# fedemagnani/optimization-solvers

Measured on AMD Instinct MI355X. Metric: BFGS iterations/sec on n-dim convex quadratic (f64) at 1/2/4/8 MI355X, higher is better.
Workload: dtype f64

## Files before the change

include/qn_hip.h:

```cpp
#ifndef QN_HIP_H
#define QN_HIP_H

#include <stddef.h>
#include <stdint.h>

#ifdef __cplusplus
extern "C" {
#endif

#define QN_ABI_VERSION 5

typedef enum {
    QN_OK = 0,
    QN_MAX_ITER_REACHED = 1,
    QN_OUT_OF_DOMAIN = 2,
    QN_ERROR_INPUT_PARAMS = 3,
    QN_ABNORMAL_TERMINATION = 4
} qn_status;

const char* qn_status_string(int status);
const char* qn_last_error_message(void);
int qn_abi_version(void);

typedef struct qn_context qn_context;
// ... 84 lines not shown
enum { QN_BFGS = 0, QN_DFP = 1, QN_GRADIENT_DESCENT = 2, QN_NEWTON = 3 ,
       QN_SR1 = 4 ,
       QN_SPG = 5 ,
       QN_PROJECTED_GRADIENT = 6 ,
       QN_PROJECTED_NEWTON = 7 ,
       QN_SPECTRAL_PROJECTED_NEWTON = 8 ,
       QN_BROYDEN = 9 ,
       QN_COORDINATE_DESCENT = 10 ,
       QN_PNORM_DESCENT = 11 ,
       QN_LBFGS = 12  };
#define QN_LBFGS_MAX_M 32
typedef struct qn_solver qn_solver;

int qn_solver_create(qn_context* ctx, int method, double tol, const double* x0_host, size_t n, qn_solver** out);
void qn_solver_destroy(qn_solver* s);
int qn_solver_set_bounds(qn_solver* s, const double* lower_bound_host, const double* upper_bound_host);
int qn_solver_set_spg_lambdas(qn_solver* s, double lambda_min, double lambda_max);
int qn_solver_spg_lambda(qn_solver* s, double* out, int* is_some);
int qn_solver_newton_factorisations(qn_solver* s, size_t* out);
int qn_solver_set_lbfgs_memory(qn_solver* s, size_t m);
int qn_solver_lbfgs_state(qn_solver* s, size_t* m, size_t* stored, double* gamma, size_t* resets);
int qn_solver_set_inverse_p(qn_solver* s, const double* p_colmajor_host);
int qn_solver_get_inverse_p(qn_solver* s, double* out_colmajor_host);
int qn_solver_reset(qn_solver* s, const double* x0_host);

typedef void (*qn_callback_fn)(void* user, qn_solver* solver);

int qn_minimize(qn_solver* s, qn_linesearch* ls, const qn_oracle* oracle, size_t max_iter_solver,
                size_t max_iter_line_search, qn_callback_fn callback, void* callback_user);

int qn_compute_step_len(qn_context* ctx, qn_linesearch* ls, const double* x_k_host, double f_k, const double* g_k_host,
                        const double* direction_host, size_t n, const qn_oracle* oracle, size_t max_iter, double* step_out);

size_t qn_solver_n(const qn_solver* s);
size_t qn_solver_k(const qn_solver* s);
int qn_solver_set_k(qn_solver* s, size_t k);
double qn_solver_tol(const qn_solver* s);
int qn_solver_get_x(qn_solver* s, double* out_host);
int qn_solver_set_x(qn_solver* s, const double* x_host);
int qn_solver_s_norm(qn_solver* s, double* out, int* is_some);
int qn_solver_y_norm(qn_solver* s, double* out, int* is_some);
int qn_solver_next_iterate_too_close(qn_solver* s, int* out);
int qn_solver_gradient_next_iterate_too_close(qn_solver* s, int* out);
int qn_solver_decrement_squared(qn_solver* s, double* out, int* is_some);
int qn_solver_get_inv_hessian(qn_solver* s, double* out_colmajor_host, int all_ranks);
int qn_solver_set_inv_hessian(qn_solver* s, const double* h_colmajor_host);
int qn_solver_compute_direction(qn_solver* s, const double* g_host, double* d_host);
int qn_solver_secant_update(qn_solver* s, const double* s_host, const double* y_host);

#define QN_TRACE_LS_MODIFIED (1 << 30)
typedef struct {
    double f, gnorm, t, s_norm, y_norm;
    int32_t n_evals;
    int32_t ls_iters;
    int32_t ls_cases;
    int32_t updated;
} qn_trace_rec;
int qn_solver_set_trace(qn_solver* s, size_t cap, int with_x);
int qn_solver_get_trace(qn_solver* s, qn_trace_rec* out_host, size_t cap, size_t* len, double* x_trace_host);

typedef struct {
    uint64_t iterations;
    uint64_t oracle_calls;
    uint64_t oracle_evals;
    uint64_t h_passes;
    uint64_t h_bytes;
    uint64_t obj_bytes;
    uint64_t launches;
    uint64_t host_syncs;
    double   t_hpass_ms, t_eval_ms, t_ctl_ms, t_comm_ms;
    uint64_t n_hpass_timed, n_eval_timed, n_ctl_timed, n_comm_timed;
    uint64_t matrix_bytes_per_pass;
    uint64_t total_minimize_calls, total_iterations, total_oracle_calls, total_oracle_evals, total_h_passes, total_h_bytes,
        total_obj_bytes;
    uint32_t path;
    uint32_t _pad;
    double   t_hreduce_ms, t_ereduce_ms;
    uint64_t n_hreduce_timed, n_ereduce_timed;
    uint64_t total_xchg_vector, total_xchg_scalar;
    double   t_newton_ms;
    uint64_t n_newton_timed;
    uint64_t newton_lu_sync_timeouts;
    uint64_t fast_machine_steps;
} qn_stats;
#define QN_PATH_FUSED 1u
#define QN_PATH_SYM 2u
#define QN_PATH_SYM_GENERIC 4u
#define QN_PATH_PIPELINED 8u
#define QN_PATH_SYM2 16u
#define QN_PATH_TILES1 32u
#define QN_PATH_VECTOR 64u
#define QN_PATH_PNEWTON 128u
#define QN_PATH_RANK1 256u
#define QN_PATH_PNORM 512u
#define QN_PATH_LBFGS 1024u
int qn_solver_get_stats(qn_solver* s, qn_stats* out);
int qn_solver_set_profiling(qn_solver* s, int on);
int qn_solver_set_sync_mode(qn_solver* s, int sync);
int qn_solver_set_tiling(qn_solver* s, int rows_per_block, int col_splits);
typedef enum {
    QN_OPT_GENERIC_KERNELS = 1,
    QN_OPT_DEFERRED_UPDATE_STEP = 2,
    QN_OPT_SYMMETRIC_STORAGE = 3,
    QN_OPT_SECOND_GENERATION = 4,
    QN_OPT_FOLDED_ACCEPT_REDUCE = 5,
    QN_OPT_ROW_SLIVERS = 6,
    QN_OPT_EVAL_PAIR_INSTANCE = 7,
    QN_OPT_EVAL_MOVER_MULTIPLIER = 8,
    QN_OPT_TAIL_REDUCE = 9,
    QN_OPT_BOUNDED_SECOND_GENERATION = 10,
    QN_OPT_NEWTON_PIVOTED_LU = 11,
    QN_OPT_LU_PER_COLUMN_PANEL = 12,
    QN_OPT_LU_LOOKAHEAD = 13,
    QN_OPT_LU_ONE_LAUNCH_PANEL = 14,
    QN_OPT_LU_FORCE_WAIT_EXPIRY = 15,
    QN_OPT_CHUNKS_PER_TRIP = 16,
    QN_OPT_LU_SPLIT_ROLE_A = 17,
    QN_OPT_LU_SPLIT_MIN_ROWS = 18,
    QN_OPT_BTB_PROJECT_IN_EVAL = 19,
    QN_OPT_EVAL_ZIGZAG = 20,
    QN_OPT_TOUCH_H_ROWS = 21,
    QN_OPT_TOUCH_Q_ROWS = 22,
    QN_OPT_PNEWTON_REUSE_FACTOR = 23,
    QN_OPT_PNORM_NONTEMPORAL = 24,
    QN_OPT_PNORM_ROWS_PER_WAVE = 25,
    QN_OPT_LBFGS_UNIT_SCALING = 26,
    QN_OPT_MACHINE_FAST_STEPS = 27
} qn_option;
int qn_solver_set_option(qn_solver* s, int option, int value);

int qn_dev_alloc(qn_context* ctx, size_t bytes, void** out_dev);
int qn_dev_free(qn_context* ctx, void* dev);
int qn_h2d(qn_context* ctx, void* dst_dev, const void* src_host, size_t bytes);
int qn_d2h(qn_context* ctx, void* dst_host, const void* src_dev, size_t bytes);
int qn_gemv(qn_context* ctx, const double* a_dev, size_t ld, size_t nrows, size_t ncols, const double* x_dev, double* y_dev);
int qn_rank2_update(qn_context* ctx, double* h_dev, size_t ld, size_t row0, size_t nrows, size_t n, const double* s_dev,
                    const double* u_dev, double c_ss, double c_su, double c_uu);
int qn_axpy(qn_context* ctx, size_t n, const double* x_dev, double t, const double* d_dev, double* out_dev);
int qn_dot(qn_context* ctx, size_t n, const double* a_dev, const double* b_dev, double* out_host);
int qn_nrm2(qn_context* ctx, size_t n, const double* a_dev, double* out_host);

#ifdef __cplusplus
}
#endif
#endif
```

optimization-solvers_amd/_abi.py:

```python
import ctypes as C
import os

_HERE = os.path.dirname(os.path.abspath(__file__))
LIB_PATH = os.environ.get("QN_HIP_LIB") or os.path.join(_HERE, "lib", "libqn_hip.so")

OK, MAX_ITER_REACHED, OUT_OF_DOMAIN, ERROR_INPUT_PARAMS, ABNORMAL_TERMINATION = range(5)
LS_MORETHUENTE, LS_BACKTRACKING, LS_MORETHUENTE_B, LS_BACKTRACKING_B, LS_GLL_QUADRATIC = 0, 1, 2, 3, 4
LS_NO_SEARCH = 5
LS_STRONG_WOLFE = 6
ORACLE_HOST, ORACLE_DEVICE_FN, ORACLE_OBJECTIVE = 0, 1, 2
BFGS, DFP, GRADIENT_DESCENT, NEWTON, SR1, SPG, PROJECTED_GRADIENT, PROJECTED_NEWTON, SPECTRAL_PROJECTED_NEWTON = 0, 1, 2, 3, 4, 5, 6, 7, 8
BROYDEN = 9
COORDINATE_DESCENT, PNORM_DESCENT = 10, 11
LBFGS = 12
LBFGS_MAX_M = 32
UNIQUE_ID_BYTES = 128

dp = C.POINTER(C.c_double)


class LineSearchStruct(C.Structure):
    _fields_ = [("kind", C.c_int32), ("_pad", C.c_int32),
                ("c1", C.c_double), ("c2", C.c_double), ("t_min", C.c_double), ("t_max", C.c_double),
                ("delta_min", C.c_double), ("delta", C.c_double), ("delta_max", C.c_double),
                ("bt_c1", C.c_double), ("bt_beta", C.c_double),
                ("lower_bound_host", C.c_void_p), ("upper_bound_host", C.c_void_p)]


HOST_ORACLE_FN = C.CFUNCTYPE(C.c_int, C.c_void_p, dp, C.c_size_t, dp, dp)
DEVICE_ORACLE_FN = C.CFUNCTYPE(C.c_int, C.c_void_p, C.c_void_p, C.c_void_p, C.c_size_t, C.c_void_p, C.c_void_p)
CALLBACK_FN = C.CFUNCTYPE(None, C.c_void_p, C.c_void_p)
HOST_HESSIAN_FN = C.CFUNCTYPE(C.c_int, C.c_void_p, dp, C.c_size_t, dp)
HOST_ALLGATHER_FN = C.CFUNCTYPE(C.c_int, C.c_void_p, dp, dp, C.c_size_t)


class OracleStruct(C.Structure):
    _fields_ = [("kind", C.c_int32), ("memoize", C.c_int32),
                ("host_fn", C.c_void_p), ("host_user", C.c_void_p),
                ("device_fn", C.c_void_p), ("device_user", C.c_void_p),
                ("objective", C.c_void_p), ("host_hessian_fn", C.c_void_p)]


class TraceRec(C.Structure):
    _fields_ = [("f", C.c_double), ("gnorm", C.c_double), ("t", C.c_double), ("s_norm", C.c_double), ("y_norm", C.c_double),
                ("n_evals", C.c_int32), ("ls_iters", C.c_int32), ("ls_cases", C.c_int32), ("updated", C.c_int32)]


class Stats(C.Structure):
    _fields_ = [("iterations", C.c_uint64), ("oracle_calls", C.c_uint64), ("oracle_evals", C.c_uint64),
                ("h_passes", C.c_uint64), ("h_bytes", C.c_uint64), ("obj_bytes", C.c_uint64),
                ("launches", C.c_uint64), ("host_syncs", C.c_uint64),
                ("t_hpass_ms", C.c_double), ("t_eval_ms", C.c_double), ("t_ctl_ms", C.c_double), ("t_comm_ms", C.c_double),
                ("n_hpass_timed", C.c_uint64), ("n_eval_timed", C.c_uint64), ("n_ctl_timed", C.c_uint64), ("n_comm_timed", C.c_uint64),
                ("matrix_bytes_per_pass", C.c_uint64),
                ("total_minimize_calls", C.c_uint64), ("total_iterations", C.c_uint64), ("total_oracle_calls", C.c_uint64),
                ("total_oracle_evals", C.c_uint64), ("total_h_passes", C.c_uint64), ("total_h_bytes", C.c_uint64),
                ("total_obj_bytes", C.c_uint64), ("path", C.c_uint32), ("_pad", C.c_uint32),
                ("t_hreduce_ms", C.c_double), ("t_ereduce_ms", C.c_double), ("n_hreduce_timed", C.c_uint64), ("n_ereduce_timed", C.c_uint64),
                ("total_xchg_vector", C.c_uint64), ("total_xchg_scalar", C.c_uint64),
                ("t_newton_ms", C.c_double), ("n_newton_timed", C.c_uint64), ("newton_lu_sync_timeouts", C.c_uint64),
                ("fast_machine_steps", C.c_uint64)]


PATH_FUSED, PATH_SYM, PATH_SYM_GENERIC, PATH_PIPELINED, PATH_SYM2, PATH_TILES1, PATH_VECTOR, PATH_PNEWTON = 1, 2, 4, 8, 16, 32, 64, 128
PATH_RANK1 = 256
PATH_PNORM = 512
PATH_LBFGS = 1024


SYMBOLS = [
    ("qn_status_string", C.c_char_p, [C.c_int]),
    ("qn_last_error_message", C.c_char_p, []),
    ("qn_abi_version", C.c_int, []),
    ("qn_device_count", C.c_int, [C.POINTER(C.c_int)]),
    ("qn_context_create", C.c_int, [C.c_int, C.POINTER(C.c_void_p)]),
    ("qn_comm_unique_id", C.c_int, [C.c_void_p]),
    ("qn_context_create_sharded", C.c_int, [C.c_int, C.c_int, C.c_int, C.c_void_p, C.POINTER(C.c_void_p)]),
    ("qn_context_create_sharded_host_exchange", C.c_int, [C.c_int, C.c_int, C.c_int, C.c_void_p, C.c_void_p, C.POINTER(C.c_void_p)]),
    ("qn_context_destroy", None, [C.c_void_p]),
    ("qn_partition", C.c_int, [C.c_size_t, C.c_int, C.POINTER(C.c_size_t), C.POINTER(C.c_size_t)]),
    ("qn_comm_selftest", C.c_int, [C.c_void_p]),
    ("qn_context_comm_check", C.c_int, [C.c_void_p]),
    ("qn_context_exchange_probe", C.c_int, [C.c_void_p, C.c_size_t, C.c_int, C.POINTER(C.c_double)]),
    ("qn_context_event_bracket_overhead", C.c_int, [C.c_void_p, C.c_int, C.POINTER(C.c_double)]),
    ("qn_context_synchronize", C.c_int, [C.c_void_p]),
    ("qn_context_rank", C.c_int, [C.c_void_p]),
    ("qn_context_world", C.c_int, [C.c_void_p]),
    ("qn_context_stream", C.c_void_p, [C.c_void_p]),
    ("qn_context_set_host_exchange_async", C.c_int, [C.c_void_p, C.c_int]),
    ("qn_context_set_trial_vector_exchange", C.c_int, [C.c_void_p, C.c_int]),
    ("qn_context_set_allreduce", C.c_int, [C.c_void_p, C.c_int]),
    ("qn_morethuente_default", None, [C.POINTER(LineSearchStruct)]),
    ("qn_morethuente_with_deltas", C.c_int, [C.POINTER(LineSearchStruct), C.c_double, C.c_double, C.c_double]),
    ("qn_morethuente_with_t_min", C.c_int, [C.POINTER(LineSearchStruct), C.c_double]),
    ("qn_morethuente_with_t_max", C.c_int, [C.POINTER(LineSearchStruct), C.c_double]),
    ("qn_morethuente_with_c1", C.c_int, [C.POINTER(LineSearchStruct), C.c_double]),
    ("qn_morethuente_with_c2", C.c_int, [C.POINTER(LineSearchStruct), C.c_double]),
    ("qn_backtracking_new", None, [C.POINTER(LineSearchStruct), C.c_double, C.c_double]),
    ("qn_morethuente_b_new", None, [C.POINTER(LineSearchStruct)]),
    ("qn_backtracking_b_new", None, [C.POINTER(LineSearchStruct), C.c_double, C.c_double, C.c_void_p, C.c_void_p]),
    ("qn_linesearch_with_lower_bound", None, [C.POINTER(LineSearchStruct), C.c_void_p]),
    ("qn_linesearch_with_upper_bound", None, [C.POINTER(LineSearchStruct), C.c_void_p]),
    ("qn_nosearch_new", None, [C.POINTER(LineSearchStruct)]),
    ("qn_gll_quadratic_new", None, [C.POINTER(LineSearchStruct), C.c_double, C.c_size_t]),
    ("qn_gll_quadratic_with_sigmas", None, [C.POINTER(LineSearchStruct), C.c_double, C.c_double]),
    ("qn_strong_wolfe_new", None, [C.POINTER(LineSearchStruct), C.c_double, C.c_double]),
    ("qn_strong_wolfe_with_xtol", C.c_int, [C.POINTER(LineSearchStruct), C.c_double]),
    ("qn_quadratic_create", C.c_int, [C.c_void_p, C.c_size_t, dp, dp, C.POINTER(C.c_void_p)]),
    ("qn_quadratic_create_synthetic", C.c_int, [C.c_void_p, C.c_size_t, C.c_uint64, dp, dp, C.POINTER(C.c_void_p)]),
    ("qn_logsumexp_create", C.c_int, [C.c_void_p, C.c_size_t, C.c_size_t, dp, dp, C.c_double, C.POINTER(C.c_void_p)]),
    ("qn_objective_destroy", None, [C.c_void_p]),
    ("qn_objective_eval", C.c_int, [C.c_void_p, dp, dp, dp]),
    ("qn_objective_get_rows", C.c_int, [C.c_void_p, C.c_size_t, C.c_size_t, dp]),
    ("qn_objective_hessian", C.c_int, [C.c_void_p, dp, dp]),
    ("qn_solver_create", C.c_int, [C.c_void_p, C.c_int, C.c_double, dp, C.c_size_t, C.POINTER(C.c_void_p)]),
    ("qn_solver_destroy", None, [C.c_void_p]),
    ("qn_solver_reset", C.c_int, [C.c_void_p, dp]),
    ("qn_solver_set_bounds", C.c_int, [C.c_void_p, dp, dp]),
    ("qn_solver_set_inverse_p", C.c_int, [C.c_void_p, dp]),
    ("qn_solver_get_inverse_p", C.c_int, [C.c_void_p, dp]),
    ("qn_solver_set_spg_lambdas", C.c_int, [C.c_void_p, C.c_double, C.c_double]),
    ("qn_solver_spg_lambda", C.c_int, [C.c_void_p, dp, C.POINTER(C.c_int)]),
    ("qn_solver_newton_factorisations", C.c_int, [C.c_void_p, C.POINTER(C.c_size_t)]),
    ("qn_solver_set_lbfgs_memory", C.c_int, [C.c_void_p, C.c_size_t]),
    ("qn_solver_lbfgs_state", C.c_int, [C.c_void_p, C.POINTER(C.c_size_t), C.POINTER(C.c_size_t), dp, C.POINTER(C.c_size_t)]),
    ("qn_minimize", C.c_int, [C.c_void_p, C.POINTER(LineSearchStruct), C.POINTER(OracleStruct), C.c_size_t, C.c_size_t, C.c_void_p, C.c_void_p]),
    ("qn_compute_step_len", C.c_int, [C.c_void_p, C.POINTER(LineSearchStruct), dp, C.c_double, dp, dp, C.c_size_t, C.POINTER(OracleStruct), C.c_size_t,
                             C.POINTER(C.c_double)]),
    ("qn_solver_n", C.c_size_t, [C.c_void_p]),
    ("qn_solver_k", C.c_size_t, [C.c_void_p]),
    ("qn_solver_set_k", C.c_int, [C.c_void_p, C.c_size_t]),
    ("qn_solver_tol", C.c_double, [C.c_void_p]),
    ("qn_solver_get_x", C.c_int, [C.c_void_p, dp]),
    ("qn_solver_set_x", C.c_int, [C.c_void_p, dp]),
    ("qn_solver_s_norm", C.c_int, [C.c_void_p, dp, C.POINTER(C.c_int)]),
    ("qn_solver_y_norm", C.c_int, [C.c_void_p, dp, C.POINTER(C.c_int)]),
    ("qn_solver_next_iterate_too_close", C.c_int, [C.c_void_p, C.POINTER(C.c_int)]),
    ("qn_solver_gradient_next_iterate_too_close", C.c_int, [C.c_void_p, C.POINTER(C.c_int)]),
    ("qn_solver_decrement_squared", C.c_int, [C.c_void_p, dp, C.POINTER(C.c_int)]),
    ("qn_solver_get_inv_hessian", C.c_int, [C.c_void_p, dp, C.c_int]),
    ("qn_solver_set_inv_hessian", C.c_int, [C.c_void_p, dp]),
    ("qn_solver_compute_direction", C.c_int, [C.c_void_p, dp, dp]),
    ("qn_solver_secant_update", C.c_int, [C.c_void_p, dp, dp]),
    ("qn_solver_set_trace", C.c_int, [C.c_void_p, C.c_size_t, C.c_int]),
# ... 37 lines not shown
```

optimization-solvers_amd/csrc/qn_ctl.h:

```cpp
#pragma once
#include <stdint.h>

enum QnPhase : int32_t {
    QN_PH_IDLE = 0,
    QN_PH_REQ_EVAL = 1,
    QN_PH_REQ_HPASS = 2,
    QN_PH_ITER_DONE = 3,
    QN_PH_DONE = 4,
    QN_PH_REQ_HPASS_EVAL = 7,
    QN_PH_REQ_VEC = 8,
    QN_PH_REQ_NEWTON = 6,
    QN_PH_REQ_DIR = 9,
    QN_PH_REQ_STEEP = 10
};

enum QnReqKind : int32_t { QN_REQ_X = 0 , QN_REQ_T = 1  };

enum QnState : int32_t {
    QN_ST_BEGIN = 0,
    QN_ST_LOOP_TOP,
    QN_ST_AFTER_EVALX,
    QN_ST_CHECK,
    QN_ST_AFTER_DIR,
    QN_ST_LS_BEGIN,
    QN_ST_MT_LOOP,
    QN_ST_MT_AFTER_T,
    QN_ST_MT_AFTER_TL,
    QN_ST_MT_AFTER_TU,
    QN_ST_MT_FINISH,
    QN_ST_BT_LOOP,
    QN_ST_BT_AFTER,
    QN_ST_AFTER_LS,
    QN_ST_AFTER_NEXT,
    QN_ST_AFTER_U,
    QN_ST_ITER_END,
    QN_ST_AFTER_NEWTON,
    QN_ST_LS_ONLY,
    QN_ST_AFTER_STEEP
};

#define QN_METHOD_BROYDEN 9
#define QN_METHOD_CD 10
#define QN_METHOD_PNORM 11
#define QN_LS_KIND_NOSEARCH 5
#define QN_LS_MODIFIED_BIT (1 << 30)

struct QnTraceRec {
    double f, gnorm, t, s_norm, y_norm;
    int32_t n_evals, ls_iters, ls_cases, updated;
};

struct QnCtl {
    double tol;
    int64_t max_iter, max_iter_ls;
    int32_t method, ls_kind, memoize, callback_mode;
    double mt_c1, mt_c2, mt_tmin, mt_tmax, mt_delta;
    double bt_c1, bt_beta;
    int64_t trace_cap;
    int32_t trace_x;
    int32_t small_n;

    int32_t phase, state, status, after_state;
    int64_t k;
    int32_t has_s_norm, has_y_norm;
    double s_norm, y_norm;
    double f_k;
    double gd0;
    double gnorm;
    double gg;
    int32_t gg_valid, xtrace_done;
    int32_t have_cur_eval;
    int32_t have_dir;

    int32_t fused, xc, sc, dir_mode, gd0_valid;
    int32_t no_defer;
    int32_t warm;
    int32_t defer_u;
    int32_t sym2;
    int32_t serviced;
    int32_t ev_par;
    int32_t ev_kind;
    double ev_t;
    double dir_ug, dir_sg;
    double st_gd0, st_yy, st_ys, st_gg, st_ss, st_dnf;
    double hp_yu, hp_ug, hp_sg;
    double hp_den;

    int32_t bounded, req_project, last_projected;
    int32_t ls_only;
    double mtb_cand;
    double bt_diff2;

    int32_t has_dec;
    int32_t s2_dir;
    double dec;

    int32_t req_kind, req_need_vectors;
    double req_t;
    int32_t hp_nrhs, hp_lazy;

    int32_t pending;
    int32_t spec_tiles;
    double c_ss, c_su, c_uu;

    double f_e, gd_e;
    int32_t last_valid, d_finite;
    double last_t, f_last, gd_last;

    int64_t ls_i;
    double t, tl, tu, ls_result;
    int32_t use_mod, conv;
    double phi_t_f, phi_t_g, psi_t_f, psi_t_g;
    double sel_f_tl, sel_g_tl, sel_f_t, sel_g_t;
    double ys;

    double tr_f, tr_gnorm;
    int32_t tr_n_evals, tr_ls_iters, tr_ls_cases, tr_ndigits, tr_updated;
    int32_t dir_ready;

    uint64_t n_oracle_calls, n_oracle_evals, n_hpasses, n_hpass_rw, n_iterations;
    uint64_t n_fast_steps;
};
```

optimization-solvers_amd/csrc/qn_ctl_step.hip.h:

```cpp
#pragma once

#ifdef QN_CTL_STAMPS
#define QN_STAMP(id) do { if (tid == 0 && V.dbg) V.dbg[stamp_base + (id)] = wall_clock64(); } while (0)
#else
#define QN_STAMP(id) do { } while (0)
#endif

#define QN_TILE_IDX(base)                                        \
    int idx[4];                                                  \
    bool ok[4];                                                  \
    _Pragma("unroll") for (int u_ = 0; u_ < 4; ++u_) {           \
        const int i_ = (base) + u_ * tpb + tid;                  \
        ok[u_] = i_ < n_pad;                                     \
        idx[u_] = ok[u_] ? i_ : 0;                               \
    }

template <int NP>
__device__ __forceinline__ void ctl_sum_partials(const double* __restrict__ part, int world, int nblk, double* lds, int wave0 = 0) {
    const int lane = threadIdx.x & 63, wave = (int)(threadIdx.x >> 6) - wave0, nw = (int)(blockDim.x >> 6) - wave0;
    if (wave < 0) return;
    for (int k = wave; k < NP; k += nw) {
        const double acc = qn_partial_col_sum(part, world, nblk, NP, k, lane);
        if (lane == 0) lds[k] = acc;
    }
}

__device__ __forceinline__ void qn_keepalive(double v) { asm volatile("" ::"v"(v)); }

__device__ __forceinline__ bool qn_check_is_scalar(const QnCtl& c) {
    return c.method != 2 && c.method != QN_METHOD_CD && c.method != QN_METHOD_PNORM && (c.small_n || c.gg_valid || c.method == 3);
}


template <int LEAN>
__device__ __forceinline__ void qn_st_begin(QnCtl& c) {
    c.k = 0;
    if (!c.warm) { c.have_cur_eval = 0; c.have_dir = 0; c.last_valid = 0; c.gg_valid = 0; }
    else c.last_valid = 0;
    c.n_oracle_calls = 0; c.n_oracle_evals = 0; c.n_hpasses = 0; c.n_hpass_rw = 0; c.n_iterations = 0;
    c.status = -1;
    c.state = QN_ST_LOOP_TOP;
}

template <int LEAN>
__device__ __forceinline__ void qn_st_loop_top(QnCtl& c) {
    if (!(c.max_iter > c.k)) {
        c.status = 1;
        c.phase = QN_PH_DONE;
    } else {
        c.tr_n_evals = 0; c.tr_ls_iters = 0; c.tr_ls_cases = 0; c.tr_ndigits = 0; c.tr_updated = 0;
        c.ls_result = NAN;
        c.n_oracle_calls++;
        c.tr_n_evals++;
        if (c.memoize && c.have_cur_eval) {
            c.state = QN_ST_CHECK;
        } else {
            c.req_kind = QN_REQ_X; c.req_t = 0.0; c.req_need_vectors = 1;
            c.after_state = QN_ST_AFTER_EVALX;
            c.phase = QN_PH_REQ_EVAL;
        }
    }
}

template <int LEAN>
__device__ __forceinline__ bool qn_st_after_evalx(QnCtl& c) {
    if (!LEAN && !c.fused) return false;
    c.f_k = c.f_e;
    c.gg = c.st_gg; c.gg_valid = 1;
    c.have_cur_eval = c.memoize;
    c.have_dir = 0;
    c.state = QN_ST_CHECK;
    return true;
}

template <int LEAN>
__device__ __forceinline__ bool qn_st_after_dir(QnCtl& c) {
    if (!LEAN && !c.fused) return false;
    c.n_hpasses++;
    if (c.pending) c.n_hpass_rw++;
    c.pending = 0;
    c.dir_mode = 0;
    c.gd0_valid = 0; c.d_finite = 0; c.last_valid = 0;
    c.state = QN_ST_LS_BEGIN;
    if (LEAN == 2 && c.s2_dir) { c.dir_ready = 0; c.after_state = QN_ST_LS_BEGIN; c.phase = QN_PH_REQ_DIR; }
    return true;
}

template <int LEAN>
__device__ __forceinline__ bool qn_st_after_next(QnCtl& c) {
    if (!LEAN && !c.fused) return false;
    c.s_norm = sqrt(c.st_ss); c.has_s_norm = 1;
    c.y_norm = sqrt(c.st_yy); c.has_y_norm = 1;
    c.ys = c.st_ys;
    c.gg = c.st_gg; c.gg_valid = 1;
    c.f_k = c.f_e;
    c.xc ^= 1;
    c.have_cur_eval = c.memoize;
    c.have_dir = 0;
    c.last_valid = 0;
    if (c.s_norm < c.tol || c.y_norm < c.tol) {
        c.state = QN_ST_ITER_END;
    } else {
        c.hp_lazy = 1; c.hp_nrhs = 2;
        const double fk = c.f_k;
        const bool will_continue = (c.k + 1 < c.max_iter) && !(isnan(fk) || isinf(fk)) && !(sqrt(c.gg) < c.tol);
        if (!LEAN && will_continue && !c.callback_mode && !c.no_defer && !c.sym2) {
            c.defer_u = 1;
            c.tr_updated = 1;
            c.have_dir = 1; c.gd0_valid = 0; c.d_finite = 0;
            c.state = QN_ST_ITER_END;
        } else {
            c.after_state = QN_ST_AFTER_U;
            c.phase = QN_PH_REQ_HPASS;
        }
    }
    return true;
}

template <int LEAN>
__device__ __forceinline__ bool qn_st_after_u(QnCtl& c) {
    if (!LEAN && !c.fused) return false;
    const double yu = c.hp_yu;
    double c_ss, c_su, c_uu;
    qn_update_coeffs(c.method, c.ys, yu, c_ss, c_su, c_uu, c.hp_den);
    c.c_ss = c_ss; c.c_su = c_su; c.c_uu = c_uu;
    c.n_hpasses++;
    if (c.pending) c.n_hpass_rw++;
    c.pending = 1;
    c.sc ^= 1;
    c.dir_mode = 1; c.dir_ug = c.hp_ug; c.dir_sg = c.hp_sg;
    c.gd0_valid = 0; c.d_finite = 0;
    c.have_dir = 1;
    if (LEAN == 2) c.dir_ready = 0;
    c.tr_updated = 1;
    c.state = QN_ST_ITER_END;
    return true;
}

template <int LEAN>
__device__ __forceinline__ bool qn_st_check(QnCtl& c, const QnVecs& V, double* small_scratch) {
    const int n = V.n, n_pad = V.n_pad;
    if (!LEAN && !qn_check_is_scalar(c)) return false;
    if (!LEAN && c.method == 3) {
        c.gnorm = c.gg_valid ? sqrt(c.gg) : NAN; c.tr_f = c.f_k; c.tr_gnorm = c.gnorm;
        const double f = c.f_k;
        if (isnan(f) || isinf(f)) { c.status = 2; c.phase = QN_PH_DONE; }
        else if (c.has_dec && c.dec * 0.5 < c.tol) { c.status = 0; c.phase = QN_PH_DONE; }
        else { c.after_state = QN_ST_AFTER_NEWTON; c.phase = QN_PH_REQ_NEWTON; }
        return true;
    }
    double gnorm, gd0 = c.gd0;
    int d_finite = c.d_finite;
    if (!LEAN && c.small_n) {
        gnorm = sqrt(ref_dot(V.g, V.g, n));
        small_direction(V.H, n_pad, n, V.g, V.d, small_scratch, V.x, c.bounded ? V.lb : nullptr, c.bounded ? V.ub : nullptr);
        if (c.ls_kind == 2) {
            double cand = INFINITY;
            for (int i = 0; i < n; ++i) {
                const double di = V.d[i];
                double v = INFINITY;
                if (di > 0.0) v = (V.lub[i] - V.x[i]) / di; else if (di < 0.0) v = (V.llb[i] - V.x[i]) / di;
                cand = fmin(v, cand);
            }
            c.mtb_cand = cand;
        }
        gd0 = ref_dot(V.g, V.d, n);
        d_finite = 1;
        for (int i = 0; i < n; ++i) d_finite &= isfinite(V.d[i]) ? 1 : 0;
    } else {
        gnorm = sqrt(c.gg);
    }
    c.gnorm = gnorm; c.tr_f = c.f_k; c.tr_gnorm = gnorm;
    const double f = c.f_k;
    if (isnan(f) || isinf(f)) {
        c.status = 2; c.phase = QN_PH_DONE;
    } else if ((c.has_s_norm && c.s_norm < c.tol) || (c.has_y_norm && c.y_norm < c.tol) || (gnorm < c.tol)) {
        c.status = 0; c.phase = QN_PH_DONE;
    } else if (!LEAN && c.small_n) {
        c.gd0 = gd0; c.d_finite = d_finite; c.last_valid = 0;
        c.state = QN_ST_LS_BEGIN;
    } else if (c.have_dir) {
        c.state = QN_ST_LS_BEGIN;
        if (LEAN == 2 && c.s2_dir) {
            if (!c.dir_ready) { c.after_state = QN_ST_LS_BEGIN; c.phase = QN_PH_REQ_DIR; }
            else if (c.s2_dir & 2) c.mt_tmax = fmin(c.mt_tmax, c.mtb_cand);
        }
    } else {
        c.hp_nrhs = 1; c.hp_lazy = 0;
        c.after_state = QN_ST_AFTER_DIR;
        c.phase = QN_PH_REQ_HPASS;
    }
    return true;
}

template <int LEAN>
__device__ __forceinline__ void qn_st_ls_begin(QnCtl& c) {
    c.ls_i = 0;
    if (!LEAN && c.ls_kind == QN_LS_KIND_NOSEARCH) { c.ls_result = 1.0; c.state = QN_ST_AFTER_LS; return; }
    if (!LEAN && c.ls_kind == 2) c.mt_tmax = fmin(c.mt_tmax, c.mtb_cand);
    if (c.ls_kind == 0 || (!LEAN && c.ls_kind == 2)) {
        c.use_mod = 0; c.conv = 0;
        c.t = fmin(fmax(1.0, c.mt_tmin), c.mt_tmax);
        c.tl = c.mt_tmin; c.tu = c.mt_tmax;
        c.state = QN_ST_MT_LOOP;
    } else {
        c.t = 1.0;
        c.state = QN_ST_BT_LOOP;
    }
}

template <int LEAN>
// ... 757 lines not shown
```

optimization-solvers_amd/csrc/qn_host_launch.hip.h:

```cpp
#pragma once
struct Run;
static int r1_enqueue_req(qn_solver* s);
static int steep_enqueue_req(qn_solver* s);
static int enqueue_newton(qn_solver* s, const qn_oracle* o, qn_objective* obj);

static int check_oracle(qn_context* c, size_t n, const qn_oracle* o, qn_objective** obj) {
    *obj = nullptr;
    if (o->kind == QN_ORACLE_HOST) return o->host_fn ? QN_OK : fail(QN_ERROR_INPUT_PARAMS, "host oracle is null");
    if (o->kind == QN_ORACLE_DEVICE_FN) return o->device_fn ? QN_OK : fail(QN_ERROR_INPUT_PARAMS, "device oracle is null");
    if (o->kind != QN_ORACLE_OBJECTIVE) return fail(QN_ERROR_INPUT_PARAMS, "unknown oracle kind");
    if (!o->objective) return fail(QN_ERROR_INPUT_PARAMS, "objective is null");
    if (o->objective->ctx != c || o->objective->n != n) return fail(QN_ERROR_INPUT_PARAMS, "objective does not match the solver");
    *obj = o->objective;
    return QN_OK;
}
static void stats_add_totals(qn_solver* s) {
    s->stats.total_minimize_calls++;
    s->stats.total_iterations += s->stats.iterations; s->stats.total_oracle_calls += s->stats.oracle_calls; s->stats.total_oracle_evals += s->stats.oracle_evals;
    s->stats.total_h_passes += s->stats.h_passes; s->stats.total_h_bytes += s->stats.h_bytes; s->stats.total_obj_bytes += s->stats.obj_bytes;
}
static int xchg_sum_or_gather(qn_context* c, double* buf, size_t cnt) { return c->use_allreduce ? exchange_sum(c, buf, cnt) : exchange(c, buf, cnt); }

struct Run {
    qn_solver* s;
// ... 256 lines not shown
                a.parity = (int)(r.s2_launches & 1);
                hipLaunchKernelGGL(s2sh_vsumt_kernel, dim3(a.nb), dim3(QN_S2_TPB), 0, c->stream, a);
                HIPCHK(hipGetLastError());
                s->stats.launches++;
            }
            ProfScope ps(s, KC_COMM);
            const XchgItem items[2] = {{half, cnt}, {s->symsh_xg, (size_t)s->T.n_pad}};
            c->n_xchg_scalar++;
            QNCHK(exchange_group(c, items, 2));
            return QN_OK;
        }
        ProfScope ps(s, KC_COMM);
        c->n_xchg_scalar++;
        QNCHK(xchg_sum_or_gather(c, half, cnt));
    }
    return QN_OK;
}
static int s2_do_vec(Run& r) {
    qn_solver* s = r.s;
    qn_context* c = s->ctx;
    if (r.s2.sh_world > 1 && c->trial_vector && !r.gobj) return s2_launch(r, QN_S2_VECD);
    if (r.s2.sh_world > 1) {
        QNCHK(s2_launch(r, QN_S2_VSUM));
        {
            ProfScope ps(s, KC_COMM);
            c->n_xchg_vector++;
            if (r.gobj) QNCHK(exchange(c, r.obj->lgall, (size_t)s->T.n_pad));
            else QNCHK(xchg_sum_or_gather(c, s->symsh_xg, (size_t)s->T.n_pad));
        }
        return s2_launch(r, QN_S2_VEC);
    }
    return s2_launch(r, r.s2.fold ? QN_S2_HTILE : QN_S2_VEC);
}
static int s2_do_hpass(Run& r, bool tiles) {
    qn_solver* s = r.s;
    qn_context* c = s->ctx;
    if (r.gobj && r.s2.sh_world == 1) {
        if (!tiles) return fail(QN_ABNORMAL_TERMINATION, "sym2 (generic objective): tiles marked done without their launch");
        QNCHK(s2_launch(r, QN_S2_GHT_A));
        QNCHK(s2g_enqueue_tiles(r));
        return s2_launch(r, QN_S2_HREDUCE);
    }
    if (tiles && r.tiles1) {
        QNCHK(s2_launch(r, QN_S2_GHT_A));
        QNCHK(s2g_enqueue_tiles(r));
    } else if (tiles) QNCHK(s2_launch(r, QN_S2_HTILE));
    if (r.s2.tred) return QN_OK;
    if (r.s2.sh_world > 1) {
        QNCHK(s2_launch(r, QN_S2_HSUM));
        ProfScope ps(s, KC_COMM);
        c->n_xchg_vector++;
        QNCHK(xchg_sum_or_gather(c, s->symsh_xg, 2 * (size_t)s->T.n_pad));
    }
    return s2_launch(r, QN_S2_HREDUCE);
}

static int s2_wait_report(Run& r, unsigned long long seq) {
    qn_solver* s = r.s;
    volatile unsigned long long* flag = s->hrep_flag;
    for (uint64_t spins = 0;; ++spins) {
        if (__atomic_load_n(flag, __ATOMIC_ACQUIRE) == seq) break;
        if ((spins & 0xfff) == 0xfff) {
            hipError_t e = hipStreamQuery(s->ctx->stream);
            if (e == hipSuccess) { if (__atomic_load_n(flag, __ATOMIC_ACQUIRE) == seq) break; return fail(QN_ABNORMAL_TERMINATION, "sym2: the batch ended without a report"); }
            if (e != hipErrorNotReady) return fail(QN_ABNORMAL_TERMINATION, std::string("sym2 batch: ") + hipGetErrorString(e));
        }
    }
    memcpy(s->hctl, s->hrep, sizeof(QnCtl));
    s->stats.host_syncs++;
    return QN_OK;
}

static int place_h(Run& r) {
    qn_solver* s = r.s;
    if (s->h_placed) return QN_OK;
    s->h_placed = true;
    const size_t np = s->T.n_pad, bytes = (size_t)s->T.rpr * np * sizeof(double);
    const char* sw = getenv("QN_H_PLACEMENT");
    if ((sw && atoi(sw) == 0) || s->ctx->world != 1 || bytes > ((size_t)330 << 20) || r.s2.fold) return QN_OK;
    hipStream_t st = s->ctx->stream;
    QnCtl* pc = s->hrep;
    memcpy(pc, s->hctl, sizeof(QnCtl));
    pc->phase = QN_PH_REQ_HPASS; pc->serviced = 0; pc->hp_nrhs = 1; pc->pending = 0; pc->after_state = QN_ST_AFTER_DIR; pc->sym2 = 1; pc->fused = 1;
    pc->spec_tiles = 0; pc->sc = 0; pc->xc = 0;
    PinnedBuf<QnCtl> pe;
    (void)pe.alloc(1, hipHostMallocMapped | hipHostMallocCoherent);
    if (pe) {
        memcpy(pe, s->hctl, sizeof(QnCtl));
        pe->phase = QN_PH_REQ_EVAL; pe->serviced = 0; pe->sym2 = 1; pe->fused = 1; pe->sc = 0; pe->xc = 0;
        pe->ev_kind = QN_REQ_T; pe->t = 1.0; pe->status = -1;
    }
    ScopedEvent e0, e1;
    if (hipEventCreate(&e0.e) != hipSuccess || hipEventCreate(&e1.e) != hipSuccess) { (void)hipGetLastError(); return QN_OK; }
    auto time_on = [&](double* H, float* out_us) -> int {
        QnS2Args a = r.s2;
        a.H = H; a.parity = 0; a.ctl_first = pc; a.rep_seq = 0;
        a.tred = 0;
        float t[6];
        for (int rep = 0; rep < 6; ++rep) {
            if (pe) {
                QnS2Args ae = a;
                ae.ctl_first = pe;
                for (int e = 0; e < 2; ++e) s2_launch_eval_plain(st, ae);
            }
            HIPCHK(hipEventRecord(e0.e, st));
            if (s->method == QN_BFGS) hipLaunchKernelGGL((s2_hpass_kernel<false, true, false>), dim3(a.G), dim3(QN_S2_TPB), 0, st, a);
            else hipLaunchKernelGGL((s2_hpass_kernel<false, false, false>), dim3(a.G), dim3(QN_S2_TPB), 0, st, a);
            HIPCHK(hipEventRecord(e1.e, st));
            HIPCHK(hipEventSynchronize(e1.e));
            float ms = 0.f;
            HIPCHK(hipEventElapsedTime(&ms, e0.e, e1.e));
            t[rep] = ms * 1e3f;
        }
        std::sort(t + 2, t + 6);
        *out_us = t[3];
        return QN_OK;
    };
    DevBuf<double> cand[2];
    struct Drain { hipStream_t st; ~Drain() { (void)hipStreamSynchronize(st); } } drained{st};
    float us[3] = {0.f, 0.f, 0.f};
    int ncand = 1, keep = 0;
    QNCHK(time_on(s->H, &us[0]));
    for (int k = 1; k < 3; ++k) {
        if (k == 2 && std::fabs(us[0] - us[1]) <= 0.06f * std::min(us[0], us[1])) break;
        if (cand[k - 1].alloc((size_t)s->T.rpr * np) != QN_OK) break;
        ++ncand;
        if (hipMemcpyAsync(cand[k - 1], s->H, bytes, hipMemcpyDeviceToDevice, st) != hipSuccess) return fail(QN_ABNORMAL_TERMINATION, "H placement: copy failed");
        QNCHK(time_on(cand[k - 1], &us[k]));
    }
    for (int k = 1; k < ncand; ++k)
        if (us[k] < 0.96f * us[keep]) keep = k;
    if (sw && atoi(sw) == 2) fprintf(stderr, "[qn] H placement: %d candidates, update kernel %.2f %.2f %.2f us, kept %d\n", ncand, us[0], us[1], us[2], keep);
    if (keep) {
        (void)hipStreamSynchronize(st);
        s->H = std::move(cand[keep - 1]);
        s->V.H = s->H;
        r.s2.H = s->H;
    }
    return QN_OK;
}

static int launch_ctl_mask(Run& r, int expect_mask) {
    qn_solver* s = r.s;
    ProfScope ps(s, KC_CTL);
    const bool hp = (expect_mask & ((1 << QN_PH_REQ_HPASS) | (1 << QN_PH_REQ_HPASS_EVAL))) != 0;
    const bool ev = (expect_mask & ((1 << QN_PH_REQ_EVAL) | (1 << QN_PH_REQ_HPASS_EVAL))) != 0;
    const dim3 blk(r.fused ? ((hp && ev) ? 768 : 576) : QN_CTL_TPB);
    QnVecs V = s->V;
    if (r.rank1) V.hcs = 1;
    if (r.oracle_tpl == QN_ORACLE_QUAD)
        hipLaunchKernelGGL(ctl_step_kernel<QN_ORACLE_QUAD>, dim3(1), blk, 0, s->ctx->stream, s->ctl, V, expect_mask);
    else
        hipLaunchKernelGGL(ctl_step_kernel<QN_ORACLE_GENERIC>, dim3(1), blk, 0, s->ctx->stream, s->ctl, V, expect_mask);
    s->stats.launches++;
    HIPCHK(hipGetLastError());
    return QN_OK;
}
static int launch_ctl(Run& r, int expect_phase) { return launch_ctl_mask(r, 1 << expect_phase); }

template <int R, int U>
static void launch_eval_fused(hipStream_t st, const QnEvalFusedArgs& a) {
    hipLaunchKernelGGL((quad_eval_fused_kernel<R, U>), dim3(a.T.rpr / R), dim3(QN_TPB), 0, st, a);
}
template <int R, int U>
static void launch_hpass_fused(hipStream_t st, const QnHPassFusedArgs& a) {
    hipLaunchKernelGGL((h_pass_fused_kernel<R, U>), dim3(a.T.rpr / R), dim3(QN_TPB), 0, st, a);
}
// ... 195 lines not shown
```

optimization-solvers_amd/csrc/qn_host_minimize.hip.h:

```cpp
#pragma once
static int vec_minimize(qn_solver* s, qn_linesearch* ls, const qn_oracle* o, size_t max_iter_solver, size_t max_iter_line_search,
                        qn_callback_fn callback, void* callback_user, int ls_only, double ls_f0);
static int vec_compute_step_len(qn_context* ctx, qn_linesearch* ls, const double* x_k_host, double f_k, const double* g_k_host,
                                const double* direction_host, size_t n, const qn_oracle* oracle, size_t max_iter, double* step_out);

static int plan_run(Run& r, qn_solver* s, qn_linesearch* ls, const qn_oracle* o, size_t max_iter_solver, size_t max_iter_line_search, double ls_f0) {
    qn_context* c = s->ctx;
    const qn_callback_fn callback = r.callback;
    const int ls_only = r.ls_only;
    if (ls->kind < QN_LS_MORETHUENTE || (ls->kind > QN_LS_BACKTRACKING_B && ls->kind != QN_LS_NO_SEARCH)) return fail(QN_ERROR_INPUT_PARAMS, "unknown line search");
    if (ls->kind == QN_LS_NO_SEARCH && s->method != QN_GRADIENT_DESCENT && s->method != QN_NEWTON && !steep_method(s->method))
        return fail(QN_ERROR_INPUT_PARAMS, "NoSearch pairs with GradientDescent, Newton, CoordinateDescent and PnormDescent only");
    if (s->method == QN_PNORM_DESCENT && !s->pnorm_set) return fail(QN_ERROR_INPUT_PARAMS, "PnormDescent: inverse_p has not been set (qn_solver_set_inverse_p)");
    if (steep_method(s->method)) QNCHK(steep_alloc(s));
    const bool ls_bounded = r.ls_bounded = ls->kind == QN_LS_MORETHUENTE_B || ls->kind == QN_LS_BACKTRACKING_B;
    if (ls_bounded || s->bounded) {
        QNCHK(bounds_alloc(s));
        if (ls_bounded) {
            QNCHK(bounds_upload(s, s->bounds_block + 2 * (size_t)s->T.n_pad, ls->lower_bound_host, -INFINITY));
            QNCHK(bounds_upload(s, s->bounds_block + 3 * (size_t)s->T.n_pad, ls->upper_bound_host, INFINITY));
        }
    }
    {
        std::vector<double> box;
        if (ls_bounded) {
            box.assign(2 * s->n, 0.0);
            for (size_t i = 0; i < s->n; ++i) { box[i] = ls->lower_bound_host ? ls->lower_bound_host[i] : -INFINITY; box[s->n + i] = ls->upper_bound_host ? ls->upper_bound_host[i] : INFINITY; }
        }
        s->ls_box_changed = ls->kind != s->last_ls_kind || box.size() != s->last_ls_box.size() ||
                            (!box.empty() && memcmp(box.data(), s->last_ls_box.data(), box.size() * sizeof(double)) != 0);
        s->last_ls_kind = ls->kind;
        s->last_ls_box.swap(box);
    }
    if (s->method == QN_NEWTON) {
        if (c->world > 1) return fail(QN_ERROR_INPUT_PARAMS, "Newton is single-GPU (SURVEY.md 8(f) row f2)");
        if (!(r.obj && (r.obj->kind == OBJ_QUADRATIC || r.obj->kind == OBJ_LOGSUMEXP)) && !(o->kind == QN_ORACLE_HOST && o->host_hessian_fn))
            return fail(QN_ERROR_INPUT_PARAMS, "Hessian not available in the oracle");
        QNCHK(newton_alloc(s));
    }

    QnCtl* h = s->hctl;
    h->tol = s->tol;
    h->max_iter = (int64_t)std::min<size_t>(max_iter_solver, (size_t)1 << 62);
    h->max_iter_ls = (int64_t)std::min<size_t>(max_iter_line_search, (size_t)1 << 62);
    h->method = s->method;
    h->ls_kind = ls->kind;
    h->memoize = o->memoize ? 1 : 0;
    h->callback_mode = callback ? 1 : 0;
    h->mt_c1 = ls->c1; h->mt_c2 = ls->c2; h->mt_tmin = ls->t_min; h->mt_tmax = ls->t_max; h->mt_delta = ls->delta;
    h->bt_c1 = ls->bt_c1; h->bt_beta = ls->bt_beta;
    h->trace_cap = (int64_t)s->trace_cap;
    h->trace_x = s->trace_x;
    h->bounded = s->bounded;
    h->req_project = 0; h->last_projected = 0; s->mtb_cand_keep = h->mtb_cand; h->mtb_cand = INFINITY;
    h->ls_only = ls_only;
    if (ls_only) { h->f_k = ls_f0; h->have_cur_eval = 0; h->have_dir = 0; h->last_valid = 0; }
    h->small_n = (s->n <= QN_SMALL_N && c->world == 1) ? 1 : 0;
    if (h->small_n && h->pending) QNCHK(flush_pending(s));
    const bool sym_base = s->T.n_pad >= 8 * QN_TB && !s->no_sym && !s->h_nonsym;
    const bool sym_ok = c->world == 1 && (s->T.n_pad % QN_TB) == 0 && sym_base;
    const bool symsh_ok = c->world > 1 && (s->T.rpr % QN_TB) == 0 && sym_base;
    const bool s2_shape = sym_ok && (size_t)s->T.n_pad == s->n && !s->no_sym2;
    const bool s2sh_shape = symsh_ok && (size_t)s->T.n_pad == s->n && !s->no_sym2 && c->world <= 64;
    const bool s2bnd_off = getenv("QN_S2_BND") && atoi(getenv("QN_S2_BND")) == 0;
    const bool s2_struct = !ls_only && s2_shape && r.obj && r.obj->q_symmetric && !s->no_s2bnd && !s2bnd_off;
    const bool s2b = (s->bounded || ls_bounded) && s2_struct;
    const bool sr1_s2 = s->method == QN_SR1 && s2_struct;
    r.fused = r.oracle_tpl == QN_ORACLE_QUAD && h->memoize && (s->method == QN_BFGS || s->method == QN_DFP || sr1_s2) && !callback && s->hcs == 1 &&
              s->qcs == 1 && !h->small_n && !s->no_fused && (!(s->bounded || ls_bounded) || s2b);
    r.gobj = r.obj && r.obj->kind == OBJ_LOGSUMEXP && r.obj->lse_kch && !r.obj->lse_two_pass && h->memoize && (s->method == QN_BFGS || s->method == QN_DFP) &&
             !callback && s->hcs == 1 && !h->small_n && !s->no_fused && !s->bounded && !ls_bounded && !ls_only &&
             (s2_shape || (s2sh_shape && (c->comm || c->host_xchg || c->host_async))) && !(getenv("QN_S2G") && atoi(getenv("QN_S2G")) == 0);
    if (r.gobj) r.fused = true;
    h->fused = r.fused ? 1 : 0;
    s->V.fused_hint = h->fused;
    r.sym = r.fused && (sym_ok || symsh_ok) && r.obj && (r.obj->q_symmetric || r.gobj);
    r.sym_generic = !r.fused && (sym_ok || symsh_ok) && s->H && s->hcs == 1 && (s->method == QN_BFGS || s->method == QN_DFP || s->method == QN_SR1);
    r.rank1 = s->method == QN_BROYDEN && !h->small_n;
    r.pnorm = s->method == QN_PNORM_DESCENT && !h->small_n;
    if (s->method == QN_BROYDEN && (r.fused || r.sym || r.sym_generic)) return fail(QN_ABNORMAL_TERMINATION, "Broyden on a symmetric-storage path");
    if ((r.sym || r.sym_generic) && c->world > 1) QNCHK(solver_alloc_symsh_lists(s));
    if (r.sym_generic) {
        if (c->world > 1) QNCHK(s->symsh_xg.ensure((size_t)c->world * 2 * s->T.n_pad, c->stream));
        const int nb = s->T.n_pad / QN_TB;
        QNCHK(s->sym_part.ensure((size_t)nb * nb * 2 * QN_TB, c->stream));
        s->sym_nb = nb;
    }
    r.sym2 = r.sym && (s2_shape || s2sh_shape);
    h->sym2 = r.sym2 ? 1 : 0;
    r.bnd = r.sym2 && (s->bounded || ls_bounded || s->method == QN_SR1);
    if ((s->bounded || ls_bounded) && r.fused && !r.bnd) return fail(QN_ABNORMAL_TERMINATION, "bounded run on a fused path that is not the second-generation one");
    if (s->method == QN_SR1 && r.fused && !r.sym2) return fail(QN_ABNORMAL_TERMINATION, "SR1 on a fused path that is not the second-generation one");
    h->s2_dir = r.bnd ? ((s->bounded ? 1 : 0) | (ls->kind == QN_LS_MORETHUENTE_B ? 2 : 0)) : 0;
    r.dirq = h->s2_dir != 0;
    r.btb = r.bnd && ls->kind == QN_LS_BACKTRACKING_B;
    r.proj = r.btb;
    if (r.bnd && ls->kind == QN_LS_MORETHUENTE_B) h->ls_kind = QN_LS_MORETHUENTE;
    {
        const size_t hhalf = c->world > 1 ? (size_t)s->T.rpr * s->T.n_pad * 8 / 2 : (size_t)s->T.n_pad * s->T.n_pad * 8 / 2;
        r.tiles1 = r.sym2 && !r.gobj && c->world > 1 && hhalf > ((size_t)320 << 20);
        if (r.sym2 && !r.gobj && getenv("QN_S2_GEN1_TILES")) r.tiles1 = atoi(getenv("QN_S2_GEN1_TILES")) != 0;
    }
    h->serviced = 0; h->ev_par = 0; h->ev_kind = QN_REQ_X; h->ev_t = 0.0; h->spec_tiles = 0;
    h->n_fast_steps = 0;
    h->defer_u = 0;
    h->no_defer = s->no_defer;
    if (!r.fused) QNCHK(fused_export(s));
    if (!(r.sym || r.sym_generic) || (s->h_diag_stale && (!r.sym2 || (r.gobj && c->world == 1) || r.tiles1))) QNCHK(ensure_full_h(s));
    if (r.fused) {
        QNCHK(solver_alloc_fused(s, r.sym));
        s->V.F.pworld = r.sym ? 1 : c->world;
        if (r.sym && c->world > 1) QNCHK(s->symsh_xg.ensure((size_t)c->world * 2 * s->T.n_pad, c->stream));
        s->V.F.b = r.gobj ? nullptr : r.obj->b;
        if (!s->fused_live) {
            const size_t vb = (size_t)s->T.n_pad * sizeof(double);
            HIPCHK(hipMemcpyAsync(s->V.F.X0, s->V.x, vb, hipMemcpyDeviceToDevice, c->stream));
            if (h->pending) {
                HIPCHK(hipMemcpyAsync(s->V.F.S0, s->V.sp, vb, hipMemcpyDeviceToDevice, c->stream));
                HIPCHK(hipMemcpyAsync(s->V.F.UN, s->V.up, vb, hipMemcpyDeviceToDevice, c->stream));
            }
            h->xc = 0; h->sc = 0;
        }
        h->warm = (s->fused_live && s->warm_obj != 0 && s->warm_obj == r.obj->serial && h->memoize && h->pending && !ls_only) ? 1 : 0;
        if (!h->warm) { h->dir_mode = 0; h->gd0_valid = 0; h->dir_ready = 0; }
        if (!r.bnd || s->ls_box_changed) h->dir_ready = 0;
        if (r.bnd && h->dir_ready) h->mtb_cand = s->mtb_cand_keep;
    } else {
        h->warm = 0;
    }
    h->phase = QN_PH_IDLE;
    h->status = -1;
    const bool can_pipeline = (r.oracle_tpl == QN_ORACLE_QUAD || r.gobj) && !callback && !(c->world > 1 && !c->comm && !c->host_async);
    r.sync = s->method == QN_NEWTON || s->method == QN_BROYDEN || steep_method(s->method) || s->sync_mode == 1 || (s->sync_mode == -1 && !(can_pipeline && o->memoize)) || !can_pipeline;
    return QN_OK;
}

static void s2_cache_policy(size_t half, int* nt, int* ntq) {
    if (2 * half <= ((size_t)230 << 20)) { *nt = 0; *ntq = 0; }
    else if (half <= ((size_t)320 << 20)) { *nt = 0; *ntq = 1; }
    else { *nt = 1; *ntq = 1; }
}

static int plan_s2_args(Run& r) {
    qn_solver* s = r.s;
    qn_context* c = s->ctx;
    QNCHK(solver_alloc_sym2(s));
    QnS2Args& a = r.s2;
    a.Q = r.obj->Q; a.H = s->H; a.n = (int)s->n; a.np = s->T.n_pad; a.nb = s->s2_nb; a.G = s->s2_G;
    a.item_ij = s->s2_items; a.maxk = s->s2_maxk; a.inorder = s->s2_inorder; a.F = s->V.F; a.part = s->sym_part;
    a.wgS = s->s2_wgS; a.trows = s->s2_trows; a.ctl2 = s->s2_ctl; a.partE = s->s2_partE;
    a.gw = r.gobj ? s->T.n_pad / 64 : 0;
    a.gmu = r.gobj ? r.obj->mu : 0.0;
    if (r.gobj && c->world > 1) QNCHK(s->s2_gws.ensure(80, c->stream));
    a.gws = s->s2_gws;
    if (r.gobj) QNCHK(s->s2_wgV.ensure((size_t)2 * s->s2_trows * QN_S2_ROW, c->stream));
    a.wgV = s->s2_wgV;
    if (r.gobj && a.gw > s->s2_trows) return fail(QN_ABNORMAL_TERMINATION, "sym2 (generic objective): more combine workgroups than table rows");
    a.fold = (s->s2_maxk <= 3 && s->s2_nb <= 32 && s->fold) ? 1 : 0;
    a.sl_first = s->s2_sl_first; a.sl_per = s->s2_sl_per;
    a.pair = (a.sl_per != 0 && s->s2_maxk == 2 && s->s2_inorder == 2 * s->s2_G && !s->no_pair) ? 1 : 0;
    if (a.sl_per && !s->h_sliver_whole) { QNCHK(ensure_full_h(s)); s->h_sliver_whole = true; }
    a.trace = s->V.trace; a.xtrace = s->V.xtrace;
    a.sh_world = c->world; a.sh_rank = c->rank; a.sh_ioff = c->rank * (s->T.rpr / QN_TB);
    a.sh_nsum = c->use_allreduce ? 1 : c->world;
    a.evS = s->s2_evS; a.xg = s->symsh_xg; a.sl_off = s->s2_sl_off; a.sl_idx = s->s2_sl_idx;
    if (c->world > 1 || r.gobj) { a.fold = 0; a.pair = 0; }
    {
        a.ring = (a.pair && s->ring && s->s2_nb * (s->s2_nb - 1) / 2 >= s->s2_G) ? 1 : 0;
        a.zig = (a.ring && s->zig) ? 1 : 0;
    }
    a.fast = (s->fast_steps && c->world == 1 && !r.gobj && !r.bnd) ? 1 : 0;
    a.projfold = (r.btb && a.pair && a.ring && !s->no_projfold) ? 1 : 0;
    if (a.projfold) r.proj = false;
    if (r.bnd) a.fold = 0;
    a.method = s->method;
    if (s->method == QN_SR1) a.fold = 0;
    a.lb = (r.bnd && s->bounded) ? s->V.lb : nullptr; a.ub = (r.bnd && s->bounded) ? s->V.ub : nullptr;
    a.llb = (r.bnd && r.ls_bounded) ? s->V.llb : nullptr; a.lub = (r.bnd && r.ls_bounded) ? s->V.lub : nullptr;
    if (r.tiles1) a.fold = 0;
    a.cnt = s->s2_cnt;
    a.cnt_stride = getenv("QN_S2_CNT_STRIDE") ? std::max(1, std::min(QN_S2_CNT_STRIDE, atoi(getenv("QN_S2_CNT_STRIDE")))) : QN_S2_CNT_STRIDE;
    const bool want_tred = getenv("QN_S2_TRED") ? atoi(getenv("QN_S2_TRED")) != 0 : s->tred;
    if (want_tred) QNCHK(s->s2_cnt.ensure((size_t)a.nb * QN_S2_CNT_STRIDE, c->stream));
    a.cnt = s->s2_cnt;
    a.tred = (c->world == 1 && !a.fold && !r.gobj && !r.tiles1 && s->s2_maxk <= QN_S2_TRED_MAXK && want_tred && s->method != QN_SR1) ? 1 : 0;
    {
        auto rows_ok = [](int v) { return v == 4 || v == 6 || v == 8 || v == 10 || v == 12 || v == 16; };
        const bool can = a.ring && !r.bnd && !a.fold && !a.tred && s->method != QN_SR1 && a.nb == 32 && a.G == 256;
        a.touch = (can && rows_ok(s->touch)) ? s->touch : 0;
        a.touchq = (can && rows_ok(s->touchq)) ? s->touchq : 0;
        a.touch_delay = std::max(0, std::min(512, s->touch_delay));
        a.touchq_delay = std::max(0, std::min(512, s->touchq_delay));
    }
    s2_cache_policy(c->world > 1 ? (size_t)s->T.rpr * s->T.n_pad * 8 / 2 : (size_t)s->T.n_pad * s->T.n_pad * 8 / 2, &a.nt, &a.ntq);
    if (getenv("QN_S2_NT")) a.nt = atoi(getenv("QN_S2_NT"));
    if (getenv("QN_S2_NTQ")) a.ntq = atoi(getenv("QN_S2_NTQ"));
    return QN_OK;
}

static int slots_needed(uint64_t evals, uint64_t iters, int cap) {
    return (int)std::min<uint64_t>((uint64_t)cap, std::max<uint64_t>(1, (evals + iters - 1) / iters));
}

static int pump_s2_sync(Run& r) {
    QnCtl* h = r.s->hctl;
    QNCHK(s2_launch(r, QN_S2_ADVANCE));
    for (;;) {
        QNCHK(s2_peek(r));
        const int ph = h->phase;
        if (ph == QN_PH_DONE) { r.status = h->status; return QN_OK; }
        const bool tiles_done = ph == QN_PH_REQ_HPASS && h->serviced == 1;
        if (h->serviced != 0 && !tiles_done) return fail(QN_ABNORMAL_TERMINATION, "sym2: request in an unexpected service state");
        if (ph == QN_PH_REQ_EVAL) QNCHK(s2_do_eval(r));
        else if (ph == QN_PH_REQ_VEC) QNCHK(s2_do_vec(r));
        else if (ph == QN_PH_REQ_DIR && r.bnd) QNCHK(s2_launch(r, QN_S2_DIR));
        else if (ph == QN_PH_REQ_HPASS) QNCHK(s2_do_hpass(r, !tiles_done));
        else return fail(QN_ABNORMAL_TERMINATION, "sym2: control block in an unexpected phase");
        QNCHK(s2_launch(r, QN_S2_ADVANCE));
    }
}

static int pump_s2_pipelined(Run& r) {
    qn_solver* s = r.s;
    qn_context* c = s->ctx;
    QnCtl* h = s->hctl;
    int slots = (r.ls->kind == QN_LS_MORETHUENTE) ? 2 : 4;
    const bool adaptive = r.s2.sh_world > 1 || r.gobj || r.bnd;
    if (adaptive) slots = s->s2_slots_hint ? s->s2_slots_hint : (r.gobj ? 1 : 2);
    bool first = true;
    uint64_t ev0 = 0, it0 = 0;
    unsigned long long seq = 0;
    for (;;) {
        if (!first) {
            QNCHK(s2_wait_report(r, seq));
            if (adaptive && h->n_iterations > it0) {
                uint64_t de = h->n_oracle_evals - ev0;
                if (it0 == 0 && !h->warm && de > 0) de -= 1;
                slots = slots_needed(de, h->n_iterations - it0, 4);
                s->s2_slots_hint = slots;
            }
            ev0 = h->n_oracle_evals; it0 = h->n_iterations;
            if (h->phase == QN_PH_DONE) { r.status = h->status; return QN_OK; }
        }
        int64_t remaining = h->max_iter - (first ? 0 : h->k);
        if (remaining < 1) remaining = 1;
        const int64_t periods = std::min<int64_t>(remaining + ((first && !h->warm) ? 1 : 0), 256);
        first = false;
        auto one_period = [&]() -> int {
            if (r.dirq) QNCHK(s2_launch(r, QN_S2_DIR));
            for (int e = 0; e < slots; ++e) QNCHK(s2_do_eval(r));
            if (r.btb) QNCHK(s2_launch(r, QN_S2_ADVANCE));
            if (!r.s2.fold && !(r.gobj && r.s2.sh_world == 1)) QNCHK(s2_do_vec(r));
            QNCHK(s2_do_hpass(r, true));
            return QN_OK;
        };
        int64_t p = 0;
        static const bool want_graph = getenv("QN_S2_GRAPH") && atoi(getenv("QN_S2_GRAPH")) != 0;
        if (want_graph && c->world == 1 && !r.gobj && !s->profiling && periods >= 3) {
            QNCHK(one_period()); ++p;
            const uint64_t l0 = r.s2_launches;
            if ((l0 & 1) != 0) { QNCHK(one_period()); ++p; }
            if (periods - p >= 2) {
                const uint64_t lbase = r.s2_launches, stat0 = s->stats.launches;
                const bool reuse = s->s2_graph_exec && memcmp(&s->s2_graph_args, &r.s2, sizeof(QnS2Args)) == 0 && s->s2_graph_slots == slots && s->s2_graph_bnd == (int)r.bnd;
                if (!reuse) {
                    if (s->s2_graph_exec) { (void)hipGraphExecDestroy(s->s2_graph_exec); s->s2_graph_exec = nullptr; }
                    hipGraph_t g = nullptr;
                    HIPCHK(hipStreamBeginCapture(c->stream, hipStreamCaptureModeThreadLocal));
                    int rc = one_period(); if (rc == QN_OK) rc = one_period();
                    const hipError_t e = hipStreamEndCapture(c->stream, &g);
                    if (rc != QN_OK) return rc;
                    HIPCHK(e);
                    HIPCHK(hipGraphInstantiate(&s->s2_graph_exec, g, nullptr, nullptr, 0));
                    (void)hipGraphDestroy(g);
                    s->s2_graph_args = r.s2; s->s2_graph_slots = slots; s->s2_graph_bnd = (int)r.bnd;
                    s->s2_graph_len = r.s2_launches - lbase; s->s2_graph_stat = s->stats.launches - stat0;
                    r.s2_launches = lbase; s->stats.launches = stat0;
                }
                if ((s->s2_graph_len & 1) == 0) {
// ... 2 lines not shown
                        r.s2_launches += s->s2_graph_len; s->stats.launches += s->s2_graph_stat;
                    }
                }
            }
        }
        for (; p < periods; ++p) QNCHK(one_period());
        seq = ++s->rep_seq;
        if (r.s2.sh_world == 1 && !r.gobj) { r.report_seq = seq; QNCHK(s2_launch(r, QN_S2_ADVANCE)); }
        else QNCHK(s2_do_eval(r, seq));
    }
}

static int pump_ctl_sync(Run& r) {
    qn_solver* s = r.s;
    QnCtl* h = s->hctl;
    QNCHK(launch_ctl(r, QN_PH_IDLE));
    for (;;) {
        QNCHK(peek_ctl(s));
        const int ph = h->phase;
        if (ph == QN_PH_DONE) { r.status = h->status; return QN_OK; }
        if (ph == QN_PH_REQ_EVAL) { QNCHK(enqueue_eval(r)); QNCHK(launch_ctl(r, QN_PH_REQ_EVAL)); }
        else if (ph == QN_PH_REQ_HPASS) { QNCHK(enqueue_hpass_req(r)); QNCHK(launch_ctl(r, QN_PH_REQ_HPASS)); }
        else if (ph == QN_PH_REQ_HPASS_EVAL) {
            QNCHK(enqueue_hpass_req(r)); QNCHK(enqueue_eval(r, 1)); QNCHK(launch_ctl(r, QN_PH_REQ_HPASS_EVAL));
        }
        else if (ph == QN_PH_REQ_NEWTON) { { ProfScope ps(s, KC_NEWTON); QNCHK(enqueue_newton(s, r.o, r.obj)); } QNCHK(launch_ctl(r, QN_PH_REQ_NEWTON)); }
        else if (ph == QN_PH_REQ_STEEP) { QNCHK(steep_enqueue_req(s)); QNCHK(launch_ctl(r, QN_PH_REQ_STEEP)); }
        else if (ph == QN_PH_ITER_DONE) { r.callback(r.callback_user, s); QNCHK(launch_ctl(r, QN_PH_ITER_DONE)); }
        else return fail(QN_ABNORMAL_TERMINATION, "control block in an unexpected phase");
    }
}

static int pump_ctl_pipelined(Run& r) {
    qn_solver* s = r.s;
    QnCtl* h = s->hctl;
    QNCHK(launch_ctl(r, QN_PH_IDLE));
    const int slots_max = (r.ls->kind == QN_LS_MORETHUENTE || r.ls->kind == QN_LS_MORETHUENTE_B) ? 2 : 4;
    int slots = slots_max;
    const bool adaptive = !r.fused;
    if (adaptive && s->gen_slots_hint) slots = std::min(slots_max, s->gen_slots_hint);
    uint64_t ev0 = 0, it0 = 0;
    bool first_batch = true;
    const int gd = s->method == QN_GRADIENT_DESCENT;
    for (;;) {
        QNCHK(peek_ctl(s));
        if (adaptive && !first_batch && h->n_iterations > it0) {
            uint64_t de = h->n_oracle_evals - ev0;
            if (it0 == 0 && de > 0) de -= 1;
            slots = slots_needed(de, h->n_iterations - it0, slots_max);
            s->gen_slots_hint = slots;
        }
        ev0 = h->n_oracle_evals; it0 = h->n_iterations;
        first_batch = false;
        if (h->phase == QN_PH_DONE) { r.status = h->status; return QN_OK; }
        int64_t remaining = h->max_iter - h->k;
        if (remaining < 1) remaining = 1;
        const int64_t periods = std::min<int64_t>(remaining, 256);
        const int first_mask = (1 << QN_PH_REQ_EVAL) | (1 << QN_PH_REQ_HPASS) | (1 << QN_PH_REQ_HPASS_EVAL);
        for (int64_t p = 0; p < periods; ++p) {
            if (r.fused) {
                QNCHK(enqueue_eval(r, 1)); QNCHK(launch_ctl_mask(r, first_mask));
                for (int e = 1; e < slots; ++e) { QNCHK(enqueue_eval(r, 0)); QNCHK(launch_ctl(r, QN_PH_REQ_EVAL)); }
                QNCHK(enqueue_hpass_req(r));
            } else {
                for (int e = 0; e < slots; ++e) { QNCHK(enqueue_eval(r)); QNCHK(launch_ctl(r, QN_PH_REQ_EVAL)); }
                if (!gd) { QNCHK(enqueue_hpass_req(r)); QNCHK(launch_ctl(r, QN_PH_REQ_HPASS)); }
            }
        }
    }
}

static void finish_stats(Run& r) {
    qn_solver* s = r.s;
    qn_context* c = s->ctx;
    QnCtl* h = s->hctl;
    if (r.fused) s->fused_live = true;
    s->warm_obj = (r.fused && r.status == QN_MAX_ITER_REACHED && h->memoize && h->have_cur_eval && h->have_dir) ? r.obj->serial : 0;
    if (r.ls->kind == QN_LS_MORETHUENTE_B) r.ls->t_max = h->mt_tmax;
    s->stats.iterations = h->n_iterations;
    s->stats.oracle_calls = h->n_oracle_calls;
    s->stats.oracle_evals = h->n_oracle_evals;
    s->stats.h_passes = h->n_hpasses;
    s->stats.fast_machine_steps = h->n_fast_steps;
    uint64_t shard = (uint64_t)s->T.rpr * (uint64_t)s->T.n_pad * 8ull;
    const uint64_t full_shard = shard;
    if (r.sym || r.sym_generic) shard = (uint64_t)s->sym_nb * (uint64_t)(s->sym_nb + 1) / 2ull * (uint64_t)QN_TB * QN_TB * 8ull;
    if ((r.sym || r.sym_generic) && c->world > 1) shard = (uint64_t)qn_symsh_ntiles(s->sym_nb, s->T.rpr / QN_TB, c->rank * (s->T.rpr / QN_TB)) * (uint64_t)QN_TB * QN_TB * 8ull;
    if (r.sym2 && !r.gobj && !r.tiles1)
        shard = (uint64_t)s->sym_nb * (uint64_t)(s->sym_nb - 1) / 2ull * (uint64_t)QN_TB * QN_TB * 8ull + (uint64_t)s->sym_nb * 73728ull;
    if (r.sym2 && c->world > 1 && !r.tiles1) {
        const uint64_t nbl = (uint64_t)(s->T.rpr / QN_TB);
        const uint64_t nt = (uint64_t)qn_symsh_ntiles(s->sym_nb, (int)nbl, c->rank * (int)nbl);
        shard = (nt - nbl) * (uint64_t)QN_TB * QN_TB * 8ull + nbl * 73728ull;
    }
    s->stats.h_bytes = (h->n_hpasses + h->n_hpass_rw) * shard;
    if (r.sym2) s->stats.h_bytes = 2 * h->n_hpasses * shard;
    s->stats.obj_bytes = (r.oracle_tpl == QN_ORACLE_QUAD) ? h->n_oracle_evals * (r.sym ? shard : full_shard) : 0;
    if (r.obj && r.obj->kind == OBJ_LOGSUMEXP)
        s->stats.obj_bytes = h->n_oracle_evals * (uint64_t)r.obj->TA.rpr * (uint64_t)r.obj->T.n_pad * 8ull * ((r.obj->lse_kch && !r.obj->lse_two_pass) ? 1ull : 2ull);
    s->stats.matrix_bytes_per_pass = shard;
    stats_add_totals(s);
    s->stats.total_xchg_vector += c->n_xchg_vector - r.xv0;
    s->stats.total_xchg_scalar += c->n_xchg_scalar - r.xs0;
    s->stats.path = (r.fused ? QN_PATH_FUSED : 0u) | (r.sym ? QN_PATH_SYM : 0u) | (r.sym_generic ? QN_PATH_SYM_GENERIC : 0u) |
                    (r.sync ? 0u : QN_PATH_PIPELINED) | (r.sym2 ? QN_PATH_SYM2 : 0u) | ((r.tiles1 || (r.gobj && c->world == 1)) ? QN_PATH_TILES1 : 0u) |
                    (r.rank1 ? QN_PATH_RANK1 : 0u) | (r.pnorm ? QN_PATH_PNORM : 0u);
}

static int minimize_impl(qn_solver* s, qn_linesearch* ls, const qn_oracle* o, size_t max_iter_solver, size_t max_iter_line_search,
                         qn_callback_fn callback, void* callback_user, int ls_only, double ls_f0) {
    if (!s || !ls || !o) return fail(QN_ERROR_INPUT_PARAMS, "null argument");
    if (vec_method(s->method)) return vec_minimize(s, ls, o, max_iter_solver, max_iter_line_search, callback, callback_user, ls_only, ls_f0);
    if (ls->kind == QN_LS_GLL_QUADRATIC) return fail(QN_ERROR_INPUT_PARAMS, "GLLQuadratic pairs with SPG / projected gradient only");
    qn_context* c = s->ctx;
    HIPCHK(hipSetDevice(c->device));
    Run r{s, o, nullptr, QN_ORACLE_GENERIC, false};
    r.ls = ls; r.callback = callback; r.callback_user = callback_user; r.ls_only = ls_only;
    r.xv0 = c->n_xchg_vector; r.xs0 = c->n_xchg_scalar;
    QNCHK(check_oracle(c, s->n, o, &r.obj));
    if (r.obj && r.obj->kind == OBJ_QUADRATIC) { r.oracle_tpl = QN_ORACLE_QUAD; s->V.b = r.obj->b; }
    else if (r.obj && r.obj->kind != OBJ_LOGSUMEXP) return fail(QN_ERROR_INPUT_PARAMS, "unsupported objective");
    QNCHK(plan_run(r, s, ls, o, max_iter_solver, max_iter_line_search, ls_f0));
    if (r.sym2) QNCHK(plan_s2_args(r));
    else QNCHK(poke_ctl(s));
    if (r.sym2 && !r.gobj) QNCHK(place_h(r));
    if (r.sym2) QNCHK(r.sync ? pump_s2_sync(r) : pump_s2_pipelined(r));
    else QNCHK(r.sync ? pump_ctl_sync(r) : pump_ctl_pipelined(r));
    finish_stats(r);
    if (c->host_async_failed) { c->host_async_failed = 0; return fail(QN_ABNORMAL_TERMINATION, "host exchange callback failed"); }
    if (r.status == QN_ABNORMAL_TERMINATION) return fail(r.status, "solver state machine aborted");
    return r.status;
}

extern "C" int qn_minimize(qn_solver* s, qn_linesearch* ls, const qn_oracle* o, size_t max_iter_solver,
                           size_t max_iter_line_search, qn_callback_fn callback, void* callback_user) {
    return minimize_impl(s, ls, o, max_iter_solver, max_iter_line_search, callback, callback_user, 0, 0.0);
}

extern "C" int qn_compute_step_len(qn_context* ctx, qn_linesearch* ls, const double* x_k_host, double f_k, const double* g_k_host,
                                   const double* direction_host, size_t n, const qn_oracle* oracle, size_t max_iter, double* step_out) {
    if (!ctx || !ls || !x_k_host || !g_k_host || !direction_host || !oracle || !step_out || n == 0)
        return fail(QN_ERROR_INPUT_PARAMS, "null argument");
    if (ls->kind == QN_LS_GLL_QUADRATIC) return vec_compute_step_len(ctx, ls, x_k_host, f_k, g_k_host, direction_host, n, oracle, max_iter, step_out);
    qn_solver* s = nullptr;
    QNCHK(qn_solver_create(ctx, QN_GRADIENT_DESCENT, 0.0, x_k_host, n, &s));
    int st = QN_OK;
    hipError_t e = hipMemcpyAsync(s->V.g, g_k_host, n * sizeof(double), hipMemcpyHostToDevice, ctx->stream);
    if (e == hipSuccess) e = hipMemcpyAsync(s->V.d, direction_host, n * sizeof(double), hipMemcpyHostToDevice, ctx->stream);
    if (e != hipSuccess) st = fail(QN_ABNORMAL_TERMINATION, std::string("compute_step_len upload: ") + hipGetErrorString(e));
    if (st == QN_OK) st = minimize_impl(s, ls, oracle, 1, max_iter, nullptr, nullptr, 1, f_k);
    if (st == QN_OK) *step_out = s->hctl->ls_result;
    qn_solver_destroy(s);
    return st;
}
```

optimization-solvers_amd/csrc/qn_host_solver.hip.h:

```cpp
#pragma once
enum { KC_HPASS = 0, KC_EVAL = 1, KC_CTL = 2, KC_COMM = 3, KC_HREDUCE = 4, KC_EREDUCE = 5, KC_NEWTON = 6 };
struct TimedEvent { hipEvent_t a, b; int cls; };
struct QnVecCtl;

struct qn_solver {
    qn_context* ctx = nullptr;
    int method = QN_BFGS;
    size_t n = 0;
    double tol = 0.0;
    QnTile T{};
    int R = 4, U = 1, hcs = 1, qcs = 1;
    DevBuf<double> H;
    DevBuf<double> vec_block;
    QnVecs V{};
    DevBuf<double> hp, q, xtrace; DevBuf<QnTraceRec> trace; DevBuf<unsigned long long> dbg;
    DevBuf<double> f_dev;
    DevBuf<double> newton_w, newton_x, newton_hsrc, newton_invl, newton_inv2;
    bool newton_big = false;
    DevBuf<double> sym_part;
    int sym_nb = 0;
    DevBuf<double> pnorm_P;
    bool pnorm_set = false;
    int pnorm_nt = -1, pnorm_rw = 0;
    DevBuf<double> steep_part;
    int steep_nshare = 0;
    DevBuf<double> r1_part;
    int r1_nb = 0;
    bool no_sym = false, h_nonsym = false;
    bool h_lower_stale = false;
    DevBuf<double> symsh_xg, symsh_gath;
    bool h_diag_stale = false;
    DevBuf<int> s2_items;
    int s2_G = 0, s2_nb = 0, s2_maxk = 0, s2_inorder = 0;
    int s2_sl_first = 0, s2_sl_per = 0, s2_sl_cfg = -1;
    bool no_sliver = false;
    bool no_pair = false;
    int ring = (getenv("QN_S2_RING") && atoi(getenv("QN_S2_RING")) == 0) ? 0 : 1;
    int zig = (getenv("QN_S2_ZIGZAG") && atoi(getenv("QN_S2_ZIGZAG")) == 0) ? 0 : 1;
    int fast_steps = 1;
    int touch = getenv("QN_S2_TOUCH") ? atoi(getenv("QN_S2_TOUCH")) : 8;
    int touchq = getenv("QN_S2_TOUCHQ") ? atoi(getenv("QN_S2_TOUCHQ")) : 6;
    int touch_delay = getenv("QN_S2_TOUCH_DELAY") ? atoi(getenv("QN_S2_TOUCH_DELAY")) : 32;
    int touchq_delay = getenv("QN_S2_TOUCHQ_DELAY") ? atoi(getenv("QN_S2_TOUCHQ_DELAY")) : 0;
    bool tred = false;
    DevBuf<int> s2_cnt;
    int gen_slots_hint = 0;
    DevBuf<double> s2_gws;
    DevBuf<double> s2_wgV;
    hipGraphExec_t s2_graph_exec = nullptr;
    QnS2Args s2_graph_args{}; int s2_graph_slots = 0, s2_graph_bnd = 0; uint64_t s2_graph_len = 0, s2_graph_stat = 0;
    int last_ls_kind = -1; std::vector<double> last_ls_box; bool ls_box_changed = false;
    double mtb_cand_keep = INFINITY;
    bool no_s2bnd = false;
    bool h_sliver_whole = false;
    DevBuf<double> s2_evS;
    DevBuf<int> s2_sl_off, s2_sl_idx;
    int s2_sl_nb = 0;
    bool h_placed = false;
    DevBuf<int> symsh_tiles;
    int s2_slots_hint = 0;
    DevBuf<double> s2_partE;
    DevBuf<double> s2_wgS;
    int s2_trows = 0;
    DevBuf<QnCtl> s2_ctl;
    bool no_sym2 = false;
    bool fold = false;
    bool fused_live = false;
    uint64_t warm_obj = 0;
    DevBuf<int> newton_fail;
    DevBuf<int> newton_piv, newton_perm;
    DevBuf<double> newton_panel;
    bool newton_lu_percol = false;
    std::vector<int> newton_piv_host;
    uint64_t newton_lu_runs = 0, newton_chol_runs = 0;
    int newton_lu_force_timeout = 0;
    int newton_lu_no_persist = 0;
    DevBuf<int> newton_sync;
    DevBuf<unsigned long long> newton_rec;
    bool no_projfold = getenv("QN_S2_PROJ_FOLD") && atoi(getenv("QN_S2_PROJ_FOLD")) == 0;
    int newton_lu_split = getenv("QN_LU_SPLIT") ? atoi(getenv("QN_LU_SPLIT")) : 4;
    int newton_lu_split_min = getenv("QN_LU_SPLIT_MIN") ? atoi(getenv("QN_LU_SPLIT_MIN")) : 4160;
    uint64_t newton_lu_sync_timeouts = 0;
    int newton_lu_timeout_fallback = 0;
    int newton_lu_no_la = 0;
    int newton_force_lu = 0;
    size_t newton_n64 = 0;
    std::vector<double> newton_hhost;
    DevBuf<QnVecCtl> vctl; PinnedBuf<QnVecCtl> hvctl;
    DevBuf<double> vpart;
    uint64_t pn_factor_serial = 0;
    int pn_reuse = 1;
    uint64_t pn_factorisations = 0;
    DevBuf<double> lb_ring, lb_part, lb_small;
    DevBuf<double> bounds_block;
    int bounded = 0;
    DevBuf<double> fused_block;
    DevBuf<double> fused_evp, fused_hpp;
    int fused_nblk = 0;
    DevBuf<QnCtl> ctl;
    PinnedBuf<unsigned char> hctl_block;
    QnCtl* hctl = nullptr;
    QnCtl* hrep = nullptr;
    unsigned long long* hrep_flag = nullptr;
    unsigned long long rep_seq = 0;
    PinnedBuf<double> hx, hg;
    size_t trace_cap = 0;
    int trace_x = 0;
    int sync_mode = -1;
    int no_fused = 0;
    int no_defer = 0;
    int profiling = 0;
    std::vector<TimedEvent> events;
    std::vector<hipEvent_t> event_pool;
    qn_stats stats{};
};

static hipEvent_t ev_get(qn_solver* s) {
    if (!s->event_pool.empty()) { hipEvent_t e = s->event_pool.back(); s->event_pool.pop_back(); return e; }
    hipEvent_t e = nullptr;
    (void)hipEventCreate(&e);
    return e;
}
struct ProfScope {
    qn_solver* s; int cls; hipEvent_t a = nullptr, b = nullptr;
    ProfScope(qn_solver* s_, int cls_) : s(s_), cls(cls_) {
        if (s->profiling && s->events.size() < 200000) { a = ev_get(s); b = ev_get(s); (void)hipEventRecord(a, s->ctx->stream); }
    }
    ~ProfScope() { if (a) { (void)hipEventRecord(b, s->ctx->stream); s->events.push_back({a, b, cls}); } }
};
static void prof_collect(qn_solver* s) {
    if (s->events.empty()) return;
    (void)hipStreamSynchronize(s->ctx->stream);
    std::vector<std::vector<float>> dur(8);
    std::vector<std::pair<int, float>> all;
    all.reserve(s->events.size());
    for (auto& e : s->events) {
        float ms = 0.f;
        const bool ok = hipEventElapsedTime(&ms, e.a, e.b) == hipSuccess;
        const int cls = (e.cls >= 0 && e.cls < 7) ? e.cls : 7;
        if (ok) { dur[cls].push_back(ms); all.push_back({e.cls, ms}); }
        s->event_pool.push_back(e.a);
        s->event_pool.push_back(e.b);
    }
    float floor_ms[8];
    for (int c = 0; c < 8; ++c) {
        floor_ms[c] = 0.f;
        if (dur[c].size() >= 8) {
            const size_t kth = dur[c].size() / 50;
            std::nth_element(dur[c].begin(), dur[c].begin() + kth, dur[c].end(), std::greater<float>());
            floor_ms[c] = 0.5f * dur[c][kth];
        }
    }
    for (auto& e : all) {
        const int cls = (e.first >= 0 && e.first < 7) ? e.first : 7;
        const float ms = e.second;
        if (ms < floor_ms[cls]) continue;
        switch (e.first) {
        case KC_HPASS: s->stats.t_hpass_ms += ms; s->stats.n_hpass_timed++; break;
        case KC_EVAL: s->stats.t_eval_ms += ms; s->stats.n_eval_timed++; break;
        case KC_CTL: s->stats.t_ctl_ms += ms; s->stats.n_ctl_timed++; break;
        case KC_HREDUCE: s->stats.t_hreduce_ms += ms; s->stats.n_hreduce_timed++; break;
        case KC_EREDUCE: s->stats.t_ereduce_ms += ms; s->stats.n_ereduce_timed++; break;
        case KC_NEWTON: s->stats.t_newton_ms += ms; s->stats.n_newton_timed++; break;
        default: s->stats.t_comm_ms += ms; s->stats.n_comm_timed++; break;
        }
    }
    s->events.clear();
}

static int solver_alloc_fused(qn_solver* s, bool sym) {
    const size_t np = s->T.n_pad;
    hipStream_t st = s->ctx->stream;
    QNCHK(s->fused_block.ensure(10 * np, st));
    const int nblk = sym ? (int)(np / QN_TB) : s->T.rpr / s->R;
    if (sym) {
        QNCHK(s->sym_part.ensure((size_t)nblk * nblk * 2 * QN_TB, st));
        s->sym_nb = nblk;
    }
    QNCHK(s->fused_evp.ensure((size_t)s->ctx->world * QN_NEVP * nblk, st));
    QNCHK(s->fused_hpp.ensure((size_t)s->ctx->world * QN_NHPP * nblk, st));
    s->fused_nblk = nblk;
    double* p = s->fused_block;
    QnFused& F = s->V.F;
    F.X0 = p; F.S0 = p + 2 * np; F.G = p + 4 * np; F.GT = p + 5 * np; F.Y = p + 6 * np;
    F.UN = p + 7 * np; F.UP = p + 8 * np; F.VV = p + 9 * np;
    F.evp = s->fused_evp; F.hpp = s->fused_hpp;
    F.nblk = nblk;
    return QN_OK;
}

static int solver_alloc_symsh_lists(qn_solver* s) {
    const int nb = s->T.n_pad / QN_TB;
    if (s->s2_sl_off && s->s2_sl_nb == nb) return QN_OK;
    const int nbl = s->T.rpr / QN_TB, ioff = s->ctx->rank * nbl;
    {
        std::vector<int> tiles;
        for (int il = 0; il < nbl; ++il)
            for (int k = 0, I = ioff + il; k < qn_symsh_cnt(I, nb); ++k) tiles.push_back((I << 16) | ((I + k) % nb));
        if (tiles.empty()) tiles.push_back(0);
        QNCHK(s->symsh_tiles.alloc(tiles.size()));
        HIPCHK(hipMemcpy(s->symsh_tiles, tiles.data(), tiles.size() * sizeof(int), hipMemcpyHostToDevice));
    }
    std::vector<int> off(nb + 1, 0), idx;
    for (int R = 0; R < nb; ++R) {
        const bool r_local = R >= ioff && R < ioff + nbl;
        for (int t = 0; t < nb; ++t) {
            const bool t_local = t >= ioff && t < ioff + nbl;
            if ((r_local && qn_symsh_owns(R, t, nb)) || (t_local && t != R && qn_symsh_owns(t, R, nb))) idx.push_back(t);
        }
        off[R + 1] = (int)idx.size();
    }
    if (idx.empty()) idx.push_back(0);
    QNCHK(s->s2_sl_off.alloc(off.size()));
    QNCHK(s->s2_sl_idx.alloc(idx.size()));
    HIPCHK(hipMemcpy(s->s2_sl_off, off.data(), off.size() * sizeof(int), hipMemcpyHostToDevice));
    HIPCHK(hipMemcpy(s->s2_sl_idx, idx.data(), idx.size() * sizeof(int), hipMemcpyHostToDevice));
    s->s2_sl_nb = nb;
    return QN_OK;
}

static int solver_alloc_sym2(qn_solver* s) {
    const int nb = s->T.n_pad / QN_TB;
    hipStream_t st = s->ctx->stream;
    const int world = s->ctx->world, rank = s->ctx->rank;
    const bool sharded = world > 1;
    const int cfg = (s->fold ? 1 : 0) | (s->no_sliver ? 2 : 0) | (sharded ? 4 : 0);
    if (s->s2_nb != nb || s->s2_sl_cfg != cfg) {
        s->s2_items.reset(); s->s2_wgS.reset(); s->s2_partE.reset(); s->s2_evS.reset(); s->s2_cnt.reset();
        s->s2_wgV.reset();
        if (s->s2_graph_exec) { (void)hipGraphExecDestroy(s->s2_graph_exec); s->s2_graph_exec = nullptr; }
        s->s2_nb = 0;
        const int nbl = s->T.rpr / QN_TB, ioff = rank * nbl;
        int nitems = nb * (nb + 1) / 2;
        int G = std::min(nitems, QN_S2_MAXG);
        if (sharded) {
            nitems = qn_symsh_ntiles(nb, nbl, ioff);
            int least = nitems;
            for (int r = 0; r < world; ++r) least = std::min(least, qn_symsh_ntiles(nb, nbl, r * nbl));
            G = std::min(least, QN_S2_MAXG);
            if (G < 1) return fail(QN_ABNORMAL_TERMINATION, "sym2: a rank without tiles");
        }
        std::vector<std::vector<int>> lists;
        int inorder = 0;
        auto deal = [&](int L) {
            lists.assign(G, std::vector<int>());
            std::vector<std::pair<double, int>> heap;
            for (int g = 0; g < G; ++g) heap.push_back({0.0, -g});
            std::make_heap(heap.begin(), heap.end());
            auto give = [&](int I, int J, double cost) {
                std::pop_heap(heap.begin(), heap.end());
                auto e = heap.back();
                lists[-e.second].push_back((I << 16) | J);
                e.first -= cost;
                heap.back() = e;
                std::push_heap(heap.begin(), heap.end());
            };
// ... 127 lines not shown
    return QN_OK;
}

extern "C" void qn_solver_destroy(qn_solver* s) {
    if (!s) return;
    (void)hipSetDevice(s->ctx->device);
    (void)hipStreamSynchronize(s->ctx->stream);
    for (auto& e : s->events) { (void)hipEventDestroy(e.a); (void)hipEventDestroy(e.b); }
    for (auto& e : s->event_pool) (void)hipEventDestroy(e);
    if (s->s2_graph_exec) (void)hipGraphExecDestroy(s->s2_graph_exec);
    delete s;
}

extern "C" int qn_solver_set_trace(qn_solver* s, size_t cap, int with_x) {
    HIPCHK(hipSetDevice(s->ctx->device));
    s->V.trace = nullptr; s->V.xtrace = nullptr; s->trace.reset(); s->xtrace.reset();
    s->trace_cap = cap;
    s->trace_x = with_x && cap;
    if (cap) {
        QNCHK(s->trace.alloc(cap));
        HIPCHK(hipMemset(s->trace, 0, cap * sizeof(QnTraceRec)));
        if (with_x) QNCHK(s->xtrace.alloc_zero(cap * s->n, s->ctx->stream));
    }
    s->V.trace = s->trace; s->V.xtrace = s->xtrace;
    return QN_OK;
}

extern "C" int qn_solver_get_trace(qn_solver* s, qn_trace_rec* out_host, size_t cap, size_t* len, double* x_trace_host) {
    HIPCHK(hipSetDevice(s->ctx->device));
    size_t m = std::min<size_t>(std::min(cap, s->trace_cap), (size_t)s->hctl->n_iterations);
    if (len) *len = m;
    static_assert(sizeof(qn_trace_rec) == sizeof(QnTraceRec), "trace record layout");
    if (m && out_host) HIPCHK(hipMemcpy(out_host, s->V.trace, m * sizeof(QnTraceRec), hipMemcpyDeviceToHost));
    if (m && x_trace_host && s->V.xtrace) HIPCHK(hipMemcpy(x_trace_host, s->V.xtrace, m * s->n * sizeof(double), hipMemcpyDeviceToHost));
    return QN_OK;
}

#if defined(QN_CTL_STAMPS) || defined(QN_S2_STAMPS)
extern "C" int qn_debug_stamps(qn_solver* s, unsigned long long* out, size_t count) {
    HIPCHK(hipSetDevice(s->ctx->device));
    if (!s->dbg) {
        QNCHK(s->dbg.alloc(1 << 20));
        HIPCHK(hipMemset(s->dbg, 0, (1 << 20) * 8));
        s->V.dbg = s->dbg;
        return QN_OK;
    }
    HIPCHK(hipStreamSynchronize(s->ctx->stream));
    HIPCHK(hipMemcpy(out, s->V.dbg, count * 8, hipMemcpyDeviceToHost));
    return QN_OK;
}
#endif

#ifdef QN_LU_STAMPS
extern "C" int qn_debug_lu_stamps(unsigned long long* out) {
    HIPCHK(hipDeviceSynchronize());
    HIPCHK(hipMemcpyFromSymbol(out, HIP_SYMBOL(qn_lu_dbg), sizeof(unsigned long long) * 64 * 16));
    return QN_OK;
}
#endif
extern "C" int qn_solver_set_profiling(qn_solver* s, int on) { s->profiling = on; return QN_OK; }
extern "C" int qn_solver_set_sync_mode(qn_solver* s, int sync) { s->sync_mode = sync; return QN_OK; }
extern "C" int qn_solver_set_option(qn_solver* s, int option, int value) {
    if (!s) return fail(QN_ERROR_INPUT_PARAMS, "null argument");
    const bool on = value != 0;
    switch (option) {
    case QN_OPT_GENERIC_KERNELS: s->no_fused = on ? 1 : 0; return QN_OK;
    case QN_OPT_DEFERRED_UPDATE_STEP: s->no_defer = on ? 0 : 1; return QN_OK;
    case QN_OPT_SYMMETRIC_STORAGE: s->no_sym = on ? 0 : 1; return QN_OK;
    case QN_OPT_SECOND_GENERATION: s->no_sym2 = on ? 0 : 1; return QN_OK;
    case QN_OPT_FOLDED_ACCEPT_REDUCE: s->fold = on ? 1 : 0; return QN_OK;
    case QN_OPT_ROW_SLIVERS: s->no_sliver = !on; return QN_OK;
    case QN_OPT_EVAL_PAIR_INSTANCE: s->no_pair = !on; return QN_OK;
    case QN_OPT_EVAL_MOVER_MULTIPLIER: s->ring = on ? 1 : 0; return QN_OK;
    case QN_OPT_TAIL_REDUCE: s->tred = on; return QN_OK;
    case QN_OPT_BOUNDED_SECOND_GENERATION: s->no_s2bnd = !on; return QN_OK;
    case QN_OPT_NEWTON_PIVOTED_LU: s->newton_force_lu = on ? 1 : 0; return QN_OK;
    case QN_OPT_LU_PER_COLUMN_PANEL: s->newton_lu_percol = on ? 1 : 0; return QN_OK;
    case QN_OPT_LU_LOOKAHEAD: s->newton_lu_no_la = on ? 0 : 1; return QN_OK;
    case QN_OPT_LU_ONE_LAUNCH_PANEL: s->newton_lu_no_persist = on ? 0 : 1; return QN_OK;
    case QN_OPT_LU_FORCE_WAIT_EXPIRY: s->newton_lu_force_timeout = on ? 1 : 0; return QN_OK;
    case QN_OPT_BTB_PROJECT_IN_EVAL: s->no_projfold = !on; return QN_OK;
    case QN_OPT_EVAL_ZIGZAG: s->zig = on ? 1 : 0; return QN_OK;
    case QN_OPT_MACHINE_FAST_STEPS: s->fast_steps = on ? 1 : 0; return QN_OK;
    case QN_OPT_PNEWTON_REUSE_FACTOR: s->pn_reuse = on ? 1 : 0; s->pn_factor_serial = 0; return QN_OK;
    case QN_OPT_LBFGS_UNIT_SCALING:
        if (s->method != QN_LBFGS) return fail(QN_ERROR_INPUT_PARAMS, "unit scaling belongs to an L-BFGS solver");
        return lbfgs_set_unit_scaling(s, on);
    case QN_OPT_PNORM_NONTEMPORAL:
        if (value < -1 || value > 1) return fail(QN_ERROR_INPUT_PARAMS, "non-temporal loads of inverse_p: 0 (plain), 1 (non-temporal) or -1 (by size)");
        s->pnorm_nt = value;
        return QN_OK;
    case QN_OPT_PNORM_ROWS_PER_WAVE:
        if (value != 0 && value != 2 && value != 4) return fail(QN_ERROR_INPUT_PARAMS, "rows per wave of the p-norm direction kernel: 2, 4 or 0 (by size)");
        s->pnorm_rw = value;
        return QN_OK;
    case QN_OPT_TOUCH_H_ROWS:
    case QN_OPT_TOUCH_Q_ROWS:
        if (value != 0 && value != 4 && value != 6 && value != 8 && value != 10 && value != 12 && value != 16) return fail(QN_ERROR_INPUT_PARAMS, "rows per wave to touch: 0, 4, 6, 8, 10, 12 or 16");
        (option == QN_OPT_TOUCH_H_ROWS ? s->touch : s->touchq) = value;
        return QN_OK;
    case QN_OPT_LU_SPLIT_ROLE_A:
        if (value != 0 && value != 1 && value != 2 && value != 4) return fail(QN_ERROR_INPUT_PARAMS, "role A runs as 1, 2 or 4 workgroups");
        s->newton_lu_split = value == 0 ? 1 : value;
        return QN_OK;
    case QN_OPT_LU_SPLIT_MIN_ROWS:
        if (value < 0) return fail(QN_ERROR_INPUT_PARAMS, "a number of rows");
        s->newton_lu_split_min = value;
        return QN_OK;
    case QN_OPT_CHUNKS_PER_TRIP:
        if (value != 1 && value != 2 && value != 4) return fail(QN_ERROR_INPUT_PARAMS, "chunks per trip must be 1, 2 or 4");
        s->U = value;
        return QN_OK;
    default: return fail(QN_ERROR_INPUT_PARAMS, "unknown option");
    }
}

extern "C" int qn_solver_set_tiling(qn_solver* s, int rows_per_block, int col_splits) {
    if (!s) return fail(QN_ERROR_INPUT_PARAMS, "null argument");
    if (rows_per_block != 0 && rows_per_block != 2 && rows_per_block != 4 && rows_per_block != 8 && rows_per_block != 16)
        return fail(QN_ERROR_INPUT_PARAMS, "rows_per_block must be 2, 4, 8 or 16 (diagnostics are named options: qn_solver_set_option)");
    if (col_splits < 0 || col_splits > 64) return fail(QN_ERROR_INPUT_PARAMS, "col_splits out of range");
    HIPCHK(hipSetDevice(s->ctx->device));
    if (rows_per_block) s->R = rows_per_block;
    if (col_splits) { s->hcs = col_splits; s->qcs = col_splits; }
    return solver_alloc_hp(s);
}

extern "C" size_t qn_solver_n(const qn_solver* s) { return s->n; }
extern "C" size_t qn_solver_k(const qn_solver* s) { return (size_t)s->hctl->k; }
extern "C" double qn_solver_tol(const qn_solver* s) { return s->tol; }

static int fused_export(qn_solver* s) {
    s->warm_obj = 0;
    if (!s->fused_live) return QN_OK;
    qn_context* c = s->ctx;
    const QnCtl* h = s->hctl;
    const size_t np = s->T.n_pad, vb = np * sizeof(double);
    HIPCHK(hipMemcpyAsync(s->V.x, s->V.F.X0 + (size_t)h->xc * np, vb, hipMemcpyDeviceToDevice, c->stream));
    if (h->pending) {
        HIPCHK(hipMemcpyAsync(s->V.sp, s->V.F.S0 + (size_t)h->sc * np, vb, hipMemcpyDeviceToDevice, c->stream));
        HIPCHK(hipMemcpyAsync(s->V.up, s->V.F.UN, vb, hipMemcpyDeviceToDevice, c->stream));
    }
    HIPCHK(hipStreamSynchronize(c->stream));
    s->fused_live = false;
    return QN_OK;
}

extern "C" int qn_solver_get_x(qn_solver* s, double* out) {
    HIPCHK(hipSetDevice(s->ctx->device));
    const double* src = s->fused_live ? s->V.F.X0 + (size_t)s->hctl->xc * (size_t)s->T.n_pad : s->V.x;
    HIPCHK(hipMemcpyAsync(out, src, s->n * sizeof(double), hipMemcpyDeviceToHost, s->ctx->stream));
    HIPCHK(hipStreamSynchronize(s->ctx->stream));
    return QN_OK;
}

static int poke_ctl(qn_solver* s) {
    HIPCHK(hipMemcpyAsync(s->ctl, s->hctl, sizeof(QnCtl), hipMemcpyHostToDevice, s->ctx->stream));
    HIPCHK(hipStreamSynchronize(s->ctx->stream));
    return QN_OK;
}
static int peek_ctl(qn_solver* s) {
    HIPCHK(hipMemcpyAsync(s->hctl, s->ctl, sizeof(QnCtl), hipMemcpyDeviceToHost, s->ctx->stream));
    HIPCHK(hipStreamSynchronize(s->ctx->stream));
    s->stats.host_syncs++;
    return QN_OK;
}

static int bounds_alloc(qn_solver* s) {
    if (s->bounds_block) return QN_OK;
    const size_t np = s->T.n_pad;
    QNCHK(s->bounds_block.alloc(4 * np));
    std::vector<double> init(4 * np);
    for (size_t i = 0; i < np; ++i) { init[i] = -INFINITY; init[np + i] = INFINITY; init[2 * np + i] = -INFINITY; init[3 * np + i] = INFINITY; }
    HIPCHK(hipMemcpy(s->bounds_block, init.data(), init.size() * sizeof(double), hipMemcpyHostToDevice));
    s->V.lb = s->bounds_block; s->V.ub = s->bounds_block + np; s->V.llb = s->bounds_block + 2 * np; s->V.lub = s->bounds_block + 3 * np;
    return QN_OK;
}
static int bounds_upload(qn_solver* s, double* dst, const double* src_host, double fill) {
    std::vector<double> v(s->T.n_pad, fill);
    if (src_host) memcpy(v.data(), src_host, s->n * sizeof(double));
    HIPCHK(hipMemcpy(dst, v.data(), v.size() * sizeof(double), hipMemcpyHostToDevice));
    return QN_OK;
}

extern "C" int qn_solver_set_bounds(qn_solver* s, const double* lb_host, const double* ub_host) {
    if (!s || !lb_host || !ub_host) return fail(QN_ERROR_INPUT_PARAMS, "null argument");
    if (s->method != QN_BFGS && s->method != QN_DFP && s->method != QN_SR1 && s->method != QN_BROYDEN && !vec_method(s->method))
        return fail(QN_ERROR_INPUT_PARAMS, "bounds need a BFGS / DFP / SR1 / Broyden / SPG / projected-gradient / L-BFGS solver");
    HIPCHK(hipSetDevice(s->ctx->device));
    QNCHK(bounds_alloc(s));
    QNCHK(bounds_upload(s, s->bounds_block, lb_host, -INFINITY));
    QNCHK(bounds_upload(s, s->bounds_block + s->T.n_pad, ub_host, INFINITY));
    std::vector<double> x(s->n);
    QNCHK(qn_solver_get_x(s, x.data()));
    for (size_t i = 0; i < s->n; ++i) x[i] = std::fmin(std::fmax(x[i], lb_host[i]), ub_host[i]);
    s->bounded = 1;
    return qn_solver_set_x(s, x.data());
}

extern "C" int qn_solver_reset(qn_solver* s, const double* x0_host) {
    if (!s || !x0_host) return fail(QN_ERROR_INPUT_PARAMS, "null argument");
    HIPCHK(hipSetDevice(s->ctx->device));
    hipStream_t st = s->ctx->stream;
    if (s->H) {
        hipLaunchKernelGGL(identity_fill_kernel, dim3(2048), dim3(256), 0, st, s->H, s->T);
        HIPCHK(hipGetLastError());
        s->h_lower_stale = false; s->h_diag_stale = false;
        s->h_nonsym = false;
    }
    s->fused_live = false; s->warm_obj = 0;
    HIPCHK(hipMemsetAsync(s->vec_block, 0, 9 * (size_t)s->T.n_pad * sizeof(double), st));
    std::vector<double> xp;
    if (vec_method(s->method) && s->bounded) {
        const size_t n = s->n;
        std::vector<double> lb(n), ub(n);
        HIPCHK(hipMemcpyAsync(lb.data(), s->bounds_block, n * sizeof(double), hipMemcpyDeviceToHost, st));
// ... 270 lines not shown
```

optimization-solvers_amd/csrc/qn_sym2.hip.h:

```cpp
#pragma once
#include <type_traits>

#define QN_S2_TPB 512
#define QN_S2_WAVES 8
#define QN_S2_RPW 16
#define QN_S2_MAXG 256
#define QN_S2_NSE 6
#define QN_S2_NR 5
#define QN_S2_ROW 8
#define QN_S2SH_NEC 4
#define QN_S2SH_EB 4
#define QN_S2_CNT_STRIDE 1056
#define QN_S2_TRED_MAXK 31

enum { QN_S2_ADVANCE = 0, QN_S2_EVAL = 1, QN_S2_VEC = 2, QN_S2_HTILE = 3, QN_S2_HREDUCE = 4,
       QN_S2_VSUM = 5, QN_S2_HSUM = 6,
       QN_S2_GEVAL_A = 7, QN_S2_GCOMB = 8, QN_S2_GHT_A = 9,
       QN_S2_DIR = 10,
       QN_S2_PROJ = 11,
       QN_S2_VECD = 12 };

struct QnS2Args {
    const double* Q;
    double* H;
    int n, np, nb, G;
    const int* item_ij;
    int maxk;
    int inorder;
    QnFused F;
    double* part;
    double* partE;
    int pair;
    int fold;
    int tred;
    int method;
    int* cnt;
    int sl_first, sl_per;
    double* wgS;
    int trows;
    QnCtl* ctl2;
    QnTraceRec* trace;
    double* xtrace;
    int parity;
    const QnCtl* ctl_first;
    QnCtl* rep;
    unsigned long long* rep_flag;
    unsigned long long rep_seq;
    int nt;
    int ntq;
    int sh_world, sh_rank;
    int sh_ioff;
    int sh_nsum;
    double* evS;
    double* xg;
    const int* sl_off;
    const int* sl_idx;
    int cnt_stride;
    double* wgV;
    int gw;
    double gmu;
    double* gws;
    const double *lb, *ub;
    const double *llb, *lub;
    int ring;
    int projfold;
    int touch, touchq;
    int touch_delay, touchq_delay;
    int zig;
    int fast;
#ifdef QN_S2_STAMPS
    unsigned long long* dbg;
    int slot;
    int swz;
#endif
};
#ifdef QN_S2_STAMPS
#define QN_S2_WG(a) ((int)blockIdx.x ^ (a).swz)
#else
#define QN_S2_WG(a) ((int)blockIdx.x)
#endif
#ifdef QN_S2_STAMPS
#define QN_S2_STAMP(k) do { if (threadIdx.x == 0 && a.dbg && blockIdx.x < 256) a.dbg[(((size_t)(a.slot & 63)) * 256 + blockIdx.x) * 16 + (k)] = wall_clock64(); } while (0)
#define QN_S2_STAMP_T(k, t) do { if (threadIdx.x == (t) && a.dbg && blockIdx.x < 256) a.dbg[(((size_t)(a.slot & 63)) * 256 + blockIdx.x) * 16 + (k)] = wall_clock64(); } while (0)
#else
#define QN_S2_STAMP(k) do { } while (0)
#define QN_S2_STAMP_T(k, t) do { } while (0)
#endif

struct QnS2Lds {
    QnCtl c;
    double red[QN_S2_WAVES][8];
    int mine;
};

template <bool BND = false>
__device__ __forceinline__ bool qn_s2_take_eval(QnCtl& c, const double* tot) {
    const double f = 0.5 * tot[0] - tot[1];
    const double gd = tot[2] - tot[3];
    c.st_gd0 = tot[4]; c.st_dnf = tot[5];
    const bool proj = BND && c.req_project != 0;
    if (c.req_kind == QN_REQ_T && !c.gd0_valid && !proj) { c.gd0 = tot[4]; c.d_finite = tot[5] == 0.0; c.gd0_valid = 1; }
    c.f_e = f; c.gd_e = gd;
    c.n_oracle_evals++;
    c.ev_par ^= 1; c.ev_kind = c.req_kind; c.ev_t = c.req_t;
    if (c.req_kind == QN_REQ_T && !proj) { c.last_valid = 1; c.last_t = c.req_t; c.f_last = f; c.gd_last = gd; }
    else c.last_valid = 0;
    if (BND) c.last_projected = proj ? 1 : 0;
    if (c.req_need_vectors) { c.phase = QN_PH_REQ_VEC; return false; }
    return true;
}
__device__ __forceinline__ void qn_s2_take_vec(QnCtl& c, const double* tot) {
    c.st_yy = tot[0]; c.st_ys = tot[1]; c.st_gg = tot[2]; c.st_ss = tot[3]; c.hp_sg = tot[4];
}
__device__ __forceinline__ void qn_s2_spec_tiles_settle(QnCtl& c) {
    if (c.spec_tiles && c.phase != QN_PH_RUNNING && c.phase != QN_PH_REQ_VEC) {
        const int ran = c.spec_tiles;
        c.spec_tiles = 0;
        if (c.phase == QN_PH_REQ_HPASS && c.serviced == 0 && c.hp_nrhs == ran) c.serviced = 1;
        else if (c.pending) { c.pending = 0; c.n_hpasses++; c.n_hpass_rw++; }
    }
}

template <bool BND = false>
__device__ __forceinline__ void qn_s2_advance(QnCtl& c, const double* tot, const QnVecs& V, const bool leader, double* scratch, const bool resume) {
    const int ph = c.phase;
    bool run = resume;
    if (!resume) {
        if (ph == QN_PH_DONE) return;
        if (ph == QN_PH_IDLE) {
            c.serviced = 0;
            c.state = c.ls_only ? QN_ST_LS_ONLY : QN_ST_BEGIN;
            c.phase = QN_PH_RUNNING;
            run = true;
        } else {
            if (c.serviced != 2) return;
            c.serviced = 0;
            if (ph == QN_PH_REQ_EVAL) {
                if (!qn_s2_take_eval<BND>(c, tot)) return;
                c.state = c.after_state;
            } else if (ph == QN_PH_REQ_VEC) {
                qn_s2_take_vec(c, tot);
                c.state = c.after_state;
            } else if (ph == QN_PH_REQ_HPASS) {
                if (c.hp_nrhs == 2) { c.hp_yu = tot[0]; c.hp_ug = tot[1]; if (BND) c.hp_den = tot[2]; }
                c.state = c.after_state;
            } else if (BND && ph == QN_PH_REQ_DIR) {
                c.mtb_cand = tot[0];
                if (c.s2_dir & 2) c.mt_tmax = fmin(c.mt_tmax, c.mtb_cand);
                c.dir_mode = 0; c.dir_ready = 1;
                c.state = c.after_state;
            } else {
                return;
            }
            c.phase = QN_PH_RUNNING;
            run = true;
        }
    }
// ... 801 lines not shown
    }
    if (wave < 2) {
        QnWaveFold<8, 32>::run(p, lane);
        if ((lane & 7) == 0) bred[wave][lane >> 3] = p[0];
    }
    __syncthreads();
    if (tid < QN_S2_NR) a.wgS[((size_t)a.parity * QN_S2_ROW + tid) * a.trows + R] = bred[0][tid] + bred[1][tid];
    QN_S2_STAMP(14);
}

template <bool SR1 = false>
__device__ __forceinline__ void qn_s2_hreduce_row(const QnS2Args& a, const int R, const int nrhs, const double tot0, const double tot1, double (*bred)[8],
                                                  const double gp, const double yv, const int half = -1, const double snew = 0.0) {
    const int tid = threadIdx.x, lane = tid & 63, wave = tid >> 6;
    if (half == 1) {
        if (tid < QN_TB && nrhs == 2) a.F.VV[R * QN_TB + tid] = tot1;
        return;
    }
    double p[8];
#pragma unroll
    for (int k = 0; k < 8; ++k) p[k] = 0.0;
    if (tid < QN_TB) {
        const int gi = R * QN_TB + tid;
        if (nrhs == 2) {
            a.F.UN[gi] = tot0;
            if (half < 0) a.F.VV[gi] = tot1;
            p[0] = yv * tot0;
            if (SR1) p[2] = (snew - tot0) * yv;
            p[1] = tot0 * gp;
        } else {
            a.F.VV[gi] = tot0;
        }
        a.F.G[gi] = gp;
    }
    if (wave < 2) {
        QnWaveFold<8, 32>::run(p, lane);
        if ((lane & 7) == 0) bred[wave][lane >> 3] = p[0];
    }
    __syncthreads();
    if (tid < (SR1 ? 3 : 2)) a.wgS[((size_t)a.parity * QN_S2_ROW + tid) * a.trows + R] = bred[0][tid] + bred[1][tid];
}
struct QnS2HReq {
    const double *sp, *up, *r0v, *gt;
    double c_ss, c_su, c_uu;
    bool pending;
};
struct QnS2HVec {
    double s_r, u_r, y0_r, y1_r;
    v2d s_c, u_c, a0, a1;
};
template <bool RHS = true>
__device__ __forceinline__ void qn_s2_hvec_load(const QnS2HReq& q, const unsigned ir, const unsigned jc, QnS2HVec& v) {
    v.s_r = q.sp[ir]; v.u_r = q.up[ir];
    v.s_c = ld2(q.sp + jc); v.u_c = ld2(q.up + jc);
    if (RHS) { v.y0_r = q.r0v[ir]; v.y1_r = q.gt[ir]; v.a0 = ld2(q.r0v + jc); v.a1 = ld2(q.gt + jc); }
}

#define QN_S2_FOLD_ITEMS 3
#define QN_S2_FOLD_BLOCKS (2 * QN_S2_FOLD_ITEMS)

template <bool NT, bool BFGS, bool FOLD, bool SHARD = false, bool TRED = false, bool SR1 = false>
__global__ __launch_bounds__(QN_S2_TPB, 2) void s2_hpass_kernel(const QnS2Args a) {
    static_assert(!(FOLD && SHARD), "the folded accept-reduce is a single-rank variant");
    static_assert(!(TRED && (FOLD || SHARD)), "the tail reduce is the single-rank kernel without the folded accept-reduce");
    static_assert(!(SR1 && (FOLD || SHARD || TRED || BFGS)), "SR1: the plain single-rank instance");
    __shared__ QnS2Lds L;
    __shared__ double colsum[2][QN_TB];
    __shared__ double colred[QN_S2_WAVES][2][QN_TB];
    __shared__ double fq[FOLD ? QN_S2_FOLD_BLOCKS : 1][4][QN_TB];
    __shared__ double fbg[FOLD ? QN_S2_FOLD_BLOCKS : 1][2][QN_TB];
    __shared__ double fv[FOLD ? QN_S2_FOLD_BLOCKS : 1][3][QN_TB];
    __shared__ double fred[2][8];
    const int tid = threadIdx.x, lane = tid & 63, wave = tid >> 6;
    const size_t np = (size_t)a.np;
    QN_S2_STAMP(0);
    int ij = qn_s2_first_item_of<SHARD>(a);
    const int ij1 = qn_s2_second_item(a);
    const int ij2 = (FOLD && ij1 >= 0 && a.maxk > 2) ? a.item_ij[(size_t)2 * a.G + blockIdx.x] : -1;
    int I = ij >> 16, J = ij & 0xffff;
    __shared__ v2d park0[QN_S2_RPW][64];
    QnS2HVec v0;
    double s1_r, y_r;
    v2d s1_c, y_c;
    auto vec_spec = [&]() {
        const int ir = I * QN_TB + wave * QN_S2_RPW + (lane & 15), jc = J * QN_TB + qn_s2_col(I == J, lane, wave);
        QnS2HReq spec;
        spec.sp = a.F.S0; spec.up = a.F.UN; spec.r0v = a.F.GT; spec.gt = a.F.GT;
        qn_s2_hvec_load<!FOLD>(spec, ir, jc, v0);
        s1_r = a.F.S0[np + ir]; s1_c = ld2(a.F.S0 + np + jc);
        if (!FOLD) { y_r = a.F.Y[ir]; y_c = ld2(a.F.Y + jc); }
    };
    if (wave == 0) qn_s2_prologue_w0<QN_S2_HTILE, SHARD>(a, L, vec_spec);
    int blk[QN_S2_FOLD_BLOCKS];
    {
        const int ijs[QN_S2_FOLD_ITEMS] = {ij, ij1 >= 0 ? ij1 : ij, ij2 >= 0 ? ij2 : ij};
#pragma unroll
        for (int k = 0; k < QN_S2_FOLD_ITEMS; ++k) { blk[2 * k] = ijs[k] >> 16; blk[2 * k + 1] = ijs[k] & 0xffff; }
    }
    double sv[QN_S2_FOLD_BLOCKS][8], sx[8], bg[QN_S2_FOLD_BLOCKS];
    if (FOLD && wave > 0) {
        const int per = (a.nb + 3) / 4;
        const int e = tid & (QN_TB - 1), qd = tid >> 7;
        const int k_lo = qd * per, k_hi = min(a.nb, k_lo + per);
#pragma unroll
        for (int b = 0; b < QN_S2_FOLD_BLOCKS; ++b) {
            const double* p = a.partE + ((size_t)blk[b] * a.nb) * QN_TB + e;
#pragma unroll
            for (int u = 0; u < 8; ++u) sv[b][u] = (k_lo + u < k_hi) ? p[(size_t)(k_lo + u) * QN_TB] : 0.0;
        }
        if (wave <= QN_S2_FOLD_BLOCKS) {
            const double* p = a.partE + ((size_t)blk[wave - 1] * a.nb) * QN_TB + lane;
#pragma unroll
            for (int u = 0; u < 8; ++u) sx[u] = (u < min(a.nb, per)) ? p[(size_t)u * QN_TB] : 0.0;
        }
        if (wave >= 4) {
            const double* src = (wave >= 6) ? a.F.G : a.F.b;
#pragma unroll
            for (int b = 0; b < QN_S2_FOLD_BLOCKS; ++b) bg[b] = src[blk[b] * QN_TB + e];
        }
    }
    v2d h[QN_S2_RPW];
    double* hbase = a.H + (size_t)(qn_s2_lrow<SHARD>(a, I) * QN_TB + wave * QN_S2_RPW) * np + (size_t)J * QN_TB + qn_s2_col(I == J, lane, wave);
    if (wave != 0) {
#pragma unroll
        for (int r = 0; r < QN_S2_RPW; ++r) h[r] = qn_sym_ld<NT>(hbase + (size_t)r * np);
        vec_spec();
        const double* q0 = a.H + (size_t)(qn_s2_lrow<SHARD>(a, I) * QN_TB) * np + (size_t)J * QN_TB + 2 * lane;
        const int r0 = (wave - 1) * 3;
        v2d t3[3];
#pragma unroll
        for (int k = 0; k < 3; ++k) t3[k] = qn_sym_ld<NT>(q0 + (size_t)min(r0 + k, QN_S2_RPW - 1) * np);
#pragma unroll
        for (int k = 0; k < 3; ++k)
            if (r0 + k < QN_S2_RPW) park0[r0 + k][lane] = t3[k];
    }
    if (FOLD && wave > 0) {
        const int e = tid & (QN_TB - 1), qd = tid >> 7;
#pragma unroll
        for (int b = 0; b < QN_S2_FOLD_BLOCKS; ++b) {
            double acc = 0.0;
#pragma unroll
            for (int u = 0; u < 8; ++u) acc = acc + sv[b][u];
            fq[b][qd][e] = acc;
        }
        if (wave <= QN_S2_FOLD_BLOCKS) {
            double acc = 0.0;
#pragma unroll
            for (int u = 0; u < 8; ++u) acc = acc + sx[u];
            fq[wave - 1][0][lane] = acc;
        }
        if (wave >= 4) {
#pragma unroll
            for (int b = 0; b < QN_S2_FOLD_BLOCKS; ++b) fbg[b][(wave - 4) >> 1][e] = bg[b];
        }
    }
    __syncthreads();
    qn_s2_ctl_out(a, L);
    const int mine = L.mine;
    if (!mine) return;
    QN_S2_STAMP(2);
    if (wave == 0) {
#pragma unroll
        for (int r = 0; r < QN_S2_RPW; ++r) h[r] = park0[r][lane];
    }
    const bool fold = FOLD && mine == 2;
    QnS2HReq q;
    bool nrhs2;
    {
        const QnCtl& c = L.c;
        q.pending = c.pending != 0;
        q.c_ss = c.c_ss; q.c_su = c.c_su; q.c_uu = c.c_uu;
        q.sp = a.F.S0 + (size_t)c.sc * np;
        q.up = a.F.UN;
        q.gt = a.F.GT;
        nrhs2 = fold ? (c.ev_kind == QN_REQ_T) : (c.hp_nrhs == 2);
        q.r0v = nrhs2 ? a.F.Y : a.F.GT;
        if (c.sc) { v0.s_r = s1_r; v0.s_c = s1_c; }
        if (!FOLD && nrhs2) { v0.y0_r = y_r; v0.a0 = y_c; }
    }
    if (FOLD) {
        if (tid < QN_TB) {
            if (fold) {
#pragma unroll
                for (int b = 0; b < QN_S2_FOLD_BLOCKS; ++b) {
                    const double qi = ((fq[b][0][tid] + fq[b][1][tid]) + fq[b][2][tid]) + fq[b][3][tid];
                    const double gti = qi - fbg[b][0][tid];
                    const double yi = gti - fbg[b][1][tid];
                    fv[b][0][tid] = nrhs2 ? yi : gti;
                    fv[b][1][tid] = gti;
                    fv[b][2][tid] = yi;
                }
            } else {
#pragma unroll
                for (int b = 0; b < QN_S2_FOLD_BLOCKS; ++b) {
                    const int gi = blk[b] * QN_TB + tid;
                    fv[b][0][tid] = q.r0v[gi];
                    fv[b][1][tid] = q.gt[gi];
                }
            }
        }
        __syncthreads();
        const int rr = wave * QN_S2_RPW + (lane & 15), cc = qn_s2_col(I == J, lane, wave);
        v0.y0_r = fv[0][0][rr]; v0.y1_r = fv[0][1][rr];
        v0.a0 = (v2d){fv[1][0][cc], fv[1][0][cc + 1]}; v0.a1 = (v2d){fv[1][1][cc], fv[1][1][cc + 1]};
    }
    const bool pend = q.pending;
    const double c_ss = pend ? q.c_ss : 0.0, c_su = pend ? q.c_su : 0.0, c_uu = pend ? q.c_uu : 0.0;
    const bool slv = !FOLD && !SHARD && a.sl_per != 0;
    auto sliver_ptr = [&]() {
        const QnS2Sliver sl = qn_s2_sliver(a, wave);
        unsigned r = sl.D * QN_TB + sl.row, c = sl.D * QN_TB + 2 * lane;
        asm volatile("" : "+v"(r), "+v"(c));
        return a.H + (size_t)r * np + c;
    };
    for (int it = 0;; ++it) {
        const bool diag = I == J;
        const double sr = pend ? v0.s_r : 0.0, ur = pend ? v0.u_r : 0.0;
        const double y0r = v0.y0_r, y1r = v0.y1_r;
        v2d sj = {0.0, 0.0}, uj = {0.0, 0.0};
        if (pend) { sj = v0.s_c; uj = v0.u_c; }
        v2d a0 = v0.a0, a1 = v0.a1;
        if (!qn_s2_row_on(diag, lane, wave)) { a0 = (v2d){0.0, 0.0}; a1 = (v2d){0.0, 0.0}; }
        int ijn = -1;
        if (it == 0) ijn = ij1;
        else if (FOLD) { if (it == 1) ijn = ij2; }
        else if (it + 1 < a.maxk) ijn = a.item_ij[(size_t)(it + 1) * a.G + blockIdx.x];
        const bool has_next = ijn >= 0;
        const int In = has_next ? (ijn >> 16) : I, Jn = has_next ? (ijn & 0xffff) : J;
        double* hnext = a.H + (size_t)(qn_s2_lrow<SHARD>(a, In) * QN_TB + wave * QN_S2_RPW) * np + (size_t)Jn * QN_TB + qn_s2_col(In == Jn, lane, wave);
        if (!has_next && slv) hnext = sliver_ptr();
        const size_t rstride = has_next ? np : 0;
        double c0x = 0.0, c0y = 0.0, c1x = 0.0, c1y = 0.0;
        double racc[QN_S2_RPW];
#pragma unroll
        for (int r = 0; r < QN_S2_RPW; ++r) {
            v2d hn = h[r];
            h[r] = qn_sym_ld<NT>(hnext + (size_t)r * rstride);
            const double si = qn_lane_bcast(sr, r), ui = qn_lane_bcast(ur, r);
            if (BFGS || SR1) {
                hn.x = hn.x + c_su * (si * uj.x + ui * sj.x);
                hn.y = hn.y + c_su * (si * uj.y + ui * sj.y);
            }
            hn.x = hn.x + c_ss * (si * sj.x);
            hn.y = hn.y + c_ss * (si * sj.y);
            if (!BFGS || SR1) {
                hn.x = hn.x + c_uu * (ui * uj.x);
                hn.y = hn.y + c_uu * (ui * uj.y);
            }
            qn_sym_st<NT>(hbase + (size_t)r * np, hn);
            const double y0 = qn_lane_bcast(y0r, r), y1 = qn_lane_bcast(y1r, r);
            double t0 = hn.x * a0.x;
            t0 = __builtin_fma(hn.y, a0.y, t0);
            double t1 = hn.x * a1.x;
            t1 = __builtin_fma(hn.y, a1.y, t1);
            {
                const auto rl = __builtin_amdgcn_permlane32_swap(__double2loint(t0), __double2loint(t1), false, false);
                const auto rh = __builtin_amdgcn_permlane32_swap(__double2hiint(t0), __double2hiint(t1), false, false);
                racc[r] = __hiloint2double(rh[0], rl[0]) + __hiloint2double(rh[1], rl[1]);
            }
            c0x = __builtin_fma(hn.x, y0, c0x);
            c0y = __builtin_fma(hn.y, y0, c0y);
            c1x = __builtin_fma(hn.x, y1, c1x);
            c1y = __builtin_fma(hn.y, y1, c1y);
        }
        if (!qn_s2_col_on(diag, lane, wave)) { c0x = 0.0; c0y = 0.0; c1x = 0.0; c1y = 0.0; }
        if (has_next) {
            const int irn = In * QN_TB + wave * QN_S2_RPW + (lane & 15), ccn = qn_s2_col(In == Jn, lane, wave);
            qn_s2_hvec_load<!FOLD>(q, irn, Jn * QN_TB + ccn, v0);
            if (FOLD) {
                const int rr = wave * QN_S2_RPW + (lane & 15), bI = 2 * (it + 1), bJ = bI + 1;
                v0.y0_r = fv[bI][0][rr]; v0.y1_r = fv[bI][1][rr];
                v0.a0 = (v2d){fv[bJ][0][ccn], fv[bJ][0][ccn + 1]}; v0.a1 = (v2d){fv[bJ][1][ccn], fv[bJ][1][ccn + 1]};
            }
        } else if (slv) {
            const QnS2Sliver sl = qn_s2_sliver(a, wave);
            unsigned r = sl.D * QN_TB + sl.row, c = sl.D * QN_TB + 2 * lane;
            asm volatile("" : "+v"(r), "+v"(c));
            qn_s2_hvec_load<true>(q, r, c, v0);
        }
        if (it == 0) { qn_keepalive(racc[0]); QN_S2_STAMP(3); QN_S2_STAMP_T(12, 448); }
        if (it == 1) { qn_keepalive(racc[0]); QN_S2_STAMP(6); QN_S2_STAMP_T(13, 448); }
        QnWaveFold<QN_S2_RPW, 16>::run(racc, lane);
        colred[wave][0][2 * lane] = c0x;
        colred[wave][0][2 * lane + 1] = c0y;
        colred[wave][1][2 * lane] = c1x;
        colred[wave][1][2 * lane + 1] = c1y;
        if ((lane & 1) == 0) {
            const int rhs = lane >> 5, rl = wave * QN_S2_RPW + ((lane >> 1) & 15);
            if (diag) colsum[rhs][rl] = racc[0];
            else qn_s2_slot_st<TRED>(a.part + (unsigned)(((I * a.nb + J) * 2 + rhs) * QN_TB + rl), racc[0]);
        }
        __syncthreads();
        if (tid < 2 * QN_TB) {
            const int crhs = tid / QN_TB, c = tid % QN_TB;
            double acc = colred[0][crhs][c];
#pragma unroll
            for (int w = 1; w < QN_S2_WAVES; ++w) acc = acc + colred[w][crhs][c];
            if (diag) qn_s2_slot_st<TRED>(a.part + (unsigned)(((I * a.nb + I) * 2 + crhs) * QN_TB + c), colsum[crhs][c] + acc);
            else qn_s2_slot_st<TRED>(a.part + (unsigned)(((J * a.nb + I) * 2 + crhs) * QN_TB + c), acc);
        }
        if (it == 0) QN_S2_STAMP(5);
        if (!has_next) break;
        I = In; J = Jn; hbase = hnext;
        __syncthreads();
    }
    if (slv) {
        v2d hn = h[0];
        const double si = pend ? v0.s_r : 0.0, ui = pend ? v0.u_r : 0.0;
        v2d sj = {0.0, 0.0}, uj = {0.0, 0.0};
        if (pend) { sj = v0.s_c; uj = v0.u_c; }
        if (BFGS || SR1) {
            hn.x = hn.x + c_su * (si * uj.x + ui * sj.x);
            hn.y = hn.y + c_su * (si * uj.y + ui * sj.y);
        }
        hn.x = hn.x + c_ss * (si * sj.x);
        hn.y = hn.y + c_ss * (si * sj.y);
        if (!BFGS || SR1) {
            hn.x = hn.x + c_uu * (ui * uj.x);
            hn.y = hn.y + c_uu * (ui * uj.y);
        }
        qn_sym_st<NT>(sliver_ptr(), hn);
        double t0 = hn.x * v0.a0.x;
        t0 = __builtin_fma(hn.y, v0.a0.y, t0);
        double t1 = hn.x * v0.a1.x;
        t1 = __builtin_fma(hn.y, v0.a1.y, t1);
        double tt[2] = {t0, t1};
        QnWaveFold<2, 32>::run(tt, lane);
        const QnS2Sliver sl = qn_s2_sliver(a, wave);
        if ((lane & 31) == 0) qn_s2_slot_st<TRED>(a.part + (unsigned)(((sl.D * a.nb + sl.D) * 2 + (lane >> 5)) * QN_TB + sl.row), tt[0]);
    }
    QN_S2_STAMP(15);
    if (TRED) {
        __shared__ int todo[2 * QN_S2_TRED_MAXK + 2];
        __shared__ double qbuf[3][QN_TB];
        asm volatile("s_waitcnt vmcnt(0)" ::: "memory");
        __syncthreads();
        QN_S2_STAMP(7);
        if (wave == 0) {
            const int k = lane >> 1;
            int R = -1;
            if (k < a.maxk) {
                const int ijk = k == 0 ? ij : (k == 1 ? ij1 : a.item_ij[(size_t)k * a.G + blockIdx.x]);
                if (ijk >= 0) {
                    const int Ik = ijk >> 16, Jk = ijk & 0xffff;
                    R = (lane & 1) ? (Jk != Ik ? Jk : -1) : Ik;
                }
            } else if (lane == 2 * a.maxk && slv) R = qn_s2_sliver(a, 0).D;
            bool last = false;
            if (R >= 0) {
                const int expect = (a.nb - 1) + ((a.sl_per != 0 && R >= a.sl_first) ? a.sl_per : 1);
                int* cp = a.cnt + (size_t)R * a.cnt_stride;
                last = __hip_atomic_fetch_add(cp, 1, __ATOMIC_RELAXED, __HIP_MEMORY_SCOPE_AGENT) + 1 == expect;
                if (last) __hip_atomic_store(cp, 0, __ATOMIC_RELAXED, __HIP_MEMORY_SCOPE_AGENT);
            }
            const unsigned long long m = __ballot(last);
            if (last) todo[1 + __popcll(m & ((1ull << lane) - 1ull))] = R;
            if (lane == 0) todo[0] = __popcll(m);
        }
        __syncthreads();
        QN_S2_STAMP(8);
        const int ntodo = todo[0];
        const int nrhs = L.c.hp_nrhs;
        for (int t = 0; t < ntodo; ++t) {
            const int R = todo[1 + t];
            QnS2Slots S0, S1;
            qn_s2_slot_issue<2, true>(a.part, a.nb, R, 0, S0);
            qn_s2_slot_issue<2, true>(a.part, a.nb, R, 1, S1);
            const double tot0 = qn_s2_slot_sum<2, true>(a.part, a.nb, R, 0, S0, qbuf);
            const double tot1 = (nrhs == 2) ? qn_s2_slot_sum<2, true>(a.part, a.nb, R, 1, S1, qbuf) : 0.0;
            double gp = 0.0, yv = 0.0;
            if (tid < QN_TB) { gp = a.F.GT[R * QN_TB + tid]; yv = a.F.Y[R * QN_TB + tid]; }
            qn_s2_hreduce_row(a, R, nrhs, tot0, tot1, fred, gp, yv);
            __syncthreads();
        }
        QN_S2_STAMP(14);
        return;
    }
    if (!fold) return;
    const QnEvalReq qe = qn_s2_eval_req<false>(L.c, true);
    const double* __restrict__ x = a.F.X0 + (size_t)qe.xc * np;
    double* __restrict__ xt = a.F.X0 + (size_t)(1 - qe.xc) * np;
    const double* __restrict__ spv = a.F.S0 + (size_t)qe.sc * np;
    double* __restrict__ sstage = a.F.S0 + (size_t)(1 - qe.sc) * np;
#pragma unroll 1
    for (int k = 0; k < QN_S2_FOLD_ITEMS; ++k) {
        const int ij_k = k == 0 ? ij : (k == 1 ? ij1 : ij2);
        if (ij_k < 0 || (ij_k >> 16) != (ij_k & 0xffff)) continue;
        const int R = ij_k >> 16;
        __syncthreads();
        if (tid < QN_TB) {
            const int gi = R * QN_TB + tid;
            const double gti = fv[2 * k][1][tid], yi = fv[2 * k][2][tid];
            double di;
            const double xi = x[gi];
            const double xti = qn_s2_trial(qe, xi, a.F.VV[gi], spv[gi], a.F.UN[gi], di);
            const double si = xti - xi;
            a.F.GT[gi] = gti;
            a.F.Y[gi] = yi;
            xt[gi] = xti;
            sstage[gi] = si;
            double p[8] = {yi * yi, yi * si, gti * gti, si * si, si * gti, 0.0, 0.0, 0.0};
            QnWaveFold<8, 32>::run(p, lane);
            if ((lane & 7) == 0) fred[wave][lane >> 3] = p[0];
        }
        __syncthreads();
        if (tid < QN_S2_NR) a.wgS[((size_t)a.parity * QN_S2_ROW + tid) * a.trows + R] = fred[0][tid] + fred[1][tid];
    }
}

template <bool SHARD = false, bool SR1 = false, int NBT = 0>
__global__ __launch_bounds__(QN_S2_TPB) void s2_hreduce_kernel(const QnS2Args a) {
    static_assert(!(SHARD && SR1), "SR1 runs on one rank");
    __shared__ QnS2Lds L;
    __shared__ double qbuf[3][QN_TB];
    __shared__ double bred[2][8];
    const int tid = threadIdx.x, wave = tid >> 6;
    const int R = SHARD ? (int)blockIdx.x : (int)(blockIdx.x >> 1), half = SHARD ? -1 : (int)(blockIdx.x & 1);
    if (NBT > 0 && __builtin_expect((int)blockIdx.x >= 2 * NBT, 0)) {
        const int b = (int)blockIdx.x - 2 * NBT;
        const int ij0 = qn_s2_item_of_index(b, NBT), ij1 = qn_s2_item_of_index(a.G + b, NBT);
        const bool flip = a.zig != 0 && ((a.parity ^ 1) & 1) != 0 && (ij1 >> 16) != (ij1 & 0xffff);
        for (int k = 0; k < a.touchq_delay; k += 8) __builtin_amdgcn_s_sleep(8);
        qn_s2_touch(a.Q, a, flip ? ij1 : ij0, a.touchq);
        return;
    }
    QnS2Slots S0;
    QN_S2_STAMP(0);
    double gp = 0.0, yv = 0.0, s0e = 0.0, s1e = 0.0;
    auto entries = [&]() {
        if (half != 1 && tid < QN_TB) {
            gp = a.F.GT[R * QN_TB + tid]; yv = a.F.Y[R * QN_TB + tid];
            if (SR1) { s0e = a.F.S0[R * QN_TB + tid]; s1e = a.F.S0[(size_t)a.np + R * QN_TB + tid]; }
        }
    };
    if (SHARD) { if (wave == 0) qn_s2_prologue_w0<QN_S2_HREDUCE, true>(a, L, entries); else entries(); }
    else if (wave == 0) qn_s2_prologue_w0<QN_S2_HREDUCE>(a, L, [&]() { qn_s2_slot_issue(a.part, a.nb, R, half, S0); entries(); });
    else { qn_s2_slot_issue(a.part, a.nb, R, half, S0); entries(); }
    __syncthreads();
    QN_S2_STAMP(2);
    qn_s2_ctl_out(a, L);
    if (!L.mine) return;
    const int nrhs = L.c.hp_nrhs;
    double tot0 = 0.0, tot1 = 0.0;
    if (!SHARD) {
        if (half == 1 && nrhs != 2) return;
        const double t = qn_s2_slot_sum(a.part, a.nb, R, half, S0, qbuf);
        if (half == 0) tot0 = t; else tot1 = t;
    } else if (tid < QN_TB) {
        const size_t np = (size_t)a.np;
        const double* xp = a.xg + (size_t)R * QN_TB + tid;
        tot0 = xp[0]; tot1 = xp[np];
        for (int r = 1; r < a.sh_nsum; ++r) { tot0 = tot0 + xp[(size_t)r * 2 * np]; tot1 = tot1 + xp[(size_t)r * 2 * np + np]; }
        if (nrhs != 2) tot1 = 0.0;
    }
    QN_S2_STAMP(13);
    qn_s2_hreduce_row<SR1>(a, R, nrhs, tot0, tot1, bred, gp, yv, half, L.c.sc ? s0e : s1e);
    QN_S2_STAMP(12);
}

template <bool WRITE>
__global__ __launch_bounds__(QN_S2_TPB, 2) void s2_place_probe_kernel(double* __restrict__ M, const int nb, const int np_, const int G, double* __restrict__ sink) {
    const int lane = threadIdx.x & 63, wave = threadIdx.x >> 6;
    const size_t np = (size_t)np_;
    const int nitems = nb * (nb + 1) / 2;
    double acc = 0.0;
#pragma unroll 1
    for (int k = 0; k < 2; ++k) {
        const int t = k * G + (int)blockIdx.x;
        if (t >= nitems) break;
        const int ij = qn_s2_item_of_index(t, nb);
        const int I = ij >> 16, J = ij & 0xffff;
        double* hb = M + (size_t)(I * QN_TB + wave * QN_S2_RPW) * np + (size_t)J * QN_TB + 2 * lane;
        v2d h[QN_S2_RPW];
#pragma unroll
        for (int r = 0; r < QN_S2_RPW; ++r) h[r] = ld2(hb + (size_t)r * np);
#pragma unroll
        for (int r = 0; r < QN_S2_RPW; ++r) {
            if (WRITE) {
                asm volatile("" : "+v"(h[r]));
                st2(hb + (size_t)r * np, h[r]);
            } else acc += h[r].x + h[r].y;
        }
    }
    if (!WRITE && acc == 12345.678) sink[blockIdx.x] = acc;
}

template <bool SHARD = false, bool GOBJ = false, int KIND = QN_S2_ADVANCE, bool BND = false>
__global__ __launch_bounds__(128) void s2_advance_kernel(const QnS2Args a) {
    __shared__ QnS2Lds L;
    if (threadIdx.x < 64) qn_s2_prologue_w0<KIND, SHARD, QnS2NoEarly, GOBJ, BND>(a, L);
    __syncthreads();
    qn_s2_ctl_out(a, L);
}

__global__ __launch_bounds__(QN_TB) void s2_dir_kernel(const QnS2Args a) {
    __shared__ QnS2Lds L;
    __shared__ double red[2];
    const int R = blockIdx.x, tid = threadIdx.x, lane = tid & 63, wave = tid >> 6;
    const int gi = R * QN_TB + tid;
    const size_t np = (size_t)a.np;
    double x0 = 0.0, x1 = 0.0, s0 = 0.0, s1 = 0.0, vv = 0.0, un = 0.0, lbi = -INFINITY, ubi = INFINITY, llbi = -INFINITY, lubi = INFINITY;
    auto entries = [&]() {
        x0 = a.F.X0[gi]; x1 = a.F.X0[np + gi]; s0 = a.F.S0[gi]; s1 = a.F.S0[np + gi]; vv = a.F.VV[gi]; un = a.F.UN[gi];
        if (a.lb) { lbi = a.lb[gi]; ubi = a.ub[gi]; }
        if (a.llb) { llbi = a.llb[gi]; lubi = a.lub[gi]; }
    };
    if (wave == 0) qn_s2_prologue_w0<QN_S2_DIR, false, decltype(entries)&, false, true>(a, L, entries);
    else entries();
    __syncthreads();
    qn_s2_ctl_out(a, L);
    if (!L.mine) return;
    const QnCtl& c = L.c;
    const double xi = c.xc ? x1 : x0, si = c.sc ? s1 : s0;
    const double al = c.c_su * c.dir_ug + c.c_ss * c.dir_sg, be = c.c_su * c.dir_sg + c.c_uu * c.dir_ug;
    const double w = c.dir_mode ? (vv + __builtin_fma(be, un, al * si)) : vv;
    double di = -w;
    if (c.s2_dir & 1) { double t = xi - w; t = fmin(fmax(t, lbi), ubi); di = t - xi; }
    a.F.VV[gi] = -di;
    double cand = INFINITY;
    if (c.s2_dir & 2) { if (di > 0.0) cand = (lubi - xi) / di; else if (di < 0.0) cand = (llbi - xi) / di; }
#pragma unroll
    for (int off = 32; off >= 1; off >>= 1) cand = fmin(cand, __shfl_xor(cand, off, 64));
    if (lane == 0) red[wave] = cand;
    __syncthreads();
    if (tid == 0) a.wgS[((size_t)a.parity * QN_S2_ROW + 0) * a.trows + R] = fmin(red[0], red[1]);
}

__global__ __launch_bounds__(QN_TB) void s2_proj_kernel(const QnS2Args a) {
// ... 44 lines not shown
```

optimization-solvers_amd/solver.py:

```python
import atexit
import ctypes as C
import weakref

import numpy as np

from . import _abi as A

_live = {"solver": weakref.WeakSet(), "objective": weakref.WeakSet(), "context": weakref.WeakSet()}


@atexit.register
def _close_all():
    for kind in ("solver", "objective", "context"):
        for obj in list(_live[kind]):
            try:
                obj.close()
            except Exception:
                pass


OPTIONS = {
    "generic_kernels": 1,
    "deferred_update_step": 2,
    "symmetric_storage": 3,
    "second_generation": 4,
    "folded_accept_reduce": 5,
    "row_slivers": 6,
    "eval_pair_instance": 7,
    "eval_mover_multiplier": 8,
    "tail_reduce": 9,
    "bounded_second_generation": 10,
    "newton_pivoted_lu": 11,
    "lu_per_column_panel": 12,
    "lu_lookahead": 13,
    "lu_one_launch_panel": 14,
    "lu_force_wait_expiry": 15,
    "chunks_per_trip": 16,
    "lu_split_role_a": 17,
    "lu_split_min_rows": 18,
    "btb_project_in_eval": 19,
    "eval_zigzag": 20,
    "touch_h_rows": 21,
    "touch_q_rows": 22,
    "pnewton_reuse_factor": 23,
    "pnorm_nontemporal": 24,
    "pnorm_rows_per_wave": 25,
    "lbfgs_unit_scaling": 26,
    "machine_fast_steps": 27,
}
OPT_GENERIC_KERNELS = 1
OPT_DEFERRED_UPDATE_STEP = 2
OPT_SYMMETRIC_STORAGE = 3
OPT_SECOND_GENERATION = 4
OPT_FOLDED_ACCEPT_REDUCE = 5
OPT_ROW_SLIVERS = 6
OPT_EVAL_PAIR_INSTANCE = 7
OPT_EVAL_MOVER_MULTIPLIER = 8
OPT_TAIL_REDUCE = 9
OPT_BOUNDED_SECOND_GENERATION = 10
OPT_NEWTON_PIVOTED_LU = 11
OPT_LU_PER_COLUMN_PANEL = 12
OPT_LU_LOOKAHEAD = 13
OPT_LU_ONE_LAUNCH_PANEL = 14
OPT_LU_FORCE_WAIT_EXPIRY = 15
OPT_CHUNKS_PER_TRIP = 16
OPT_LU_SPLIT_ROLE_A = 17
OPT_LU_SPLIT_MIN_ROWS = 18
OPT_BTB_PROJECT_IN_EVAL = 19
OPT_EVAL_ZIGZAG = 20
OPT_TOUCH_H_ROWS = 21
OPT_TOUCH_Q_ROWS = 22
OPT_PNEWTON_REUSE_FACTOR = 23
OPT_PNORM_NONTEMPORAL = 24
OPT_PNORM_ROWS_PER_WAVE = 25
OPT_LBFGS_UNIT_SCALING = 26
OPT_MACHINE_FAST_STEPS = 27


class SolverError(Exception):
    code = A.ABNORMAL_TERMINATION

    def __init__(self, msg=None):
        super().__init__(msg or A.lib().qn_status_string(self.code).decode())


class MaxIterReached(SolverError):
    code = A.MAX_ITER_REACHED


class OutOfDomain(SolverError):
    code = A.OUT_OF_DOMAIN


class ErrorInputParams(SolverError):
    code = A.ERROR_INPUT_PARAMS


class AbnormalTermination(SolverError):
    code = A.ABNORMAL_TERMINATION


_ERRORS = {A.MAX_ITER_REACHED: MaxIterReached, A.OUT_OF_DOMAIN: OutOfDomain, A.ERROR_INPUT_PARAMS: ErrorInputParams,
           A.ABNORMAL_TERMINATION: AbnormalTermination}


def _check(status):
    if status == A.OK:
        return
    detail = A.lib().qn_last_error_message().decode()
    cls = _ERRORS.get(status, AbnormalTermination)
    if status in (A.ERROR_INPUT_PARAMS, A.ABNORMAL_TERMINATION) and detail:
        raise cls(f"{A.lib().qn_status_string(status).decode()}: {detail}")
    raise cls()


def _f64(a):
    return np.ascontiguousarray(a, dtype=np.float64)


def _dp(a):
    return a.ctypes.data_as(A.dp)


class FuncEvalMultivariate:

    def __init__(self, f, g, hessian=None):
        self._f, self._g = float(f), np.asarray(g, dtype=np.float64)
        self._h = hessian

    @classmethod
    def new(cls, f, g):
        return cls(f, g)

    def with_hessian(self, hessian):
        self._h = np.asarray(hessian, dtype=np.float64)
        return self

    def hessian(self):
        return self._h

    def f(self):
        return self._f

    def g(self):
        return self._g

    def __iter__(self):
        return iter((self._f, self._g))


class Context:

    def __init__(self, device=0, rank=0, world=1, unique_id=None, host_allgather=None):
        L = A.lib()
        self.h = C.c_void_p()
        self._keep = None
        if world == 1:
            _check(L.qn_context_create(device, C.byref(self.h)))
        elif host_allgather is not None:
# ... 869 lines not shown
```

rust/src/ffi.rs:

```rust
#![allow(non_camel_case_types)]
use std::os::raw::{c_char, c_int, c_void};

pub const QN_ABI_VERSION: c_int = 5;

pub const QN_OK: c_int = 0;
pub const QN_MAX_ITER_REACHED: c_int = 1;
pub const QN_OUT_OF_DOMAIN: c_int = 2;
pub const QN_ERROR_INPUT_PARAMS: c_int = 3;
pub const QN_ABNORMAL_TERMINATION: c_int = 4;

pub const QN_LS_MORETHUENTE: i32 = 0;
pub const QN_LS_BACKTRACKING: i32 = 1;
pub const QN_LS_MORETHUENTE_B: i32 = 2;
pub const QN_LS_BACKTRACKING_B: i32 = 3;
pub const QN_LS_GLL_QUADRATIC: i32 = 4;
pub const QN_LS_NO_SEARCH: i32 = 5;
pub const QN_LS_STRONG_WOLFE: i32 = 6;

pub const QN_ORACLE_HOST: i32 = 0;
pub const QN_ORACLE_DEVICE_FN: i32 = 1;
pub const QN_ORACLE_OBJECTIVE: i32 = 2;

pub const QN_BFGS: c_int = 0;
pub const QN_DFP: c_int = 1;
pub const QN_GRADIENT_DESCENT: c_int = 2;
pub const QN_NEWTON: c_int = 3;
pub const QN_SR1: c_int = 4;
pub const QN_SPG: c_int = 5;
pub const QN_PROJECTED_GRADIENT: c_int = 6;
pub const QN_PROJECTED_NEWTON: c_int = 7;
pub const QN_SPECTRAL_PROJECTED_NEWTON: c_int = 8;
pub const QN_BROYDEN: c_int = 9;
pub const QN_COORDINATE_DESCENT: c_int = 10;
pub const QN_PNORM_DESCENT: c_int = 11;
pub const QN_LBFGS: c_int = 12;
pub const QN_LBFGS_MAX_M: usize = 32;

pub const QN_OPT_GENERIC_KERNELS: c_int = 1;
pub const QN_OPT_DEFERRED_UPDATE_STEP: c_int = 2;
pub const QN_OPT_SYMMETRIC_STORAGE: c_int = 3;
pub const QN_OPT_SECOND_GENERATION: c_int = 4;
pub const QN_OPT_FOLDED_ACCEPT_REDUCE: c_int = 5;
pub const QN_OPT_ROW_SLIVERS: c_int = 6;
pub const QN_OPT_EVAL_PAIR_INSTANCE: c_int = 7;
pub const QN_OPT_EVAL_MOVER_MULTIPLIER: c_int = 8;
pub const QN_OPT_TAIL_REDUCE: c_int = 9;
pub const QN_OPT_BOUNDED_SECOND_GENERATION: c_int = 10;
pub const QN_OPT_NEWTON_PIVOTED_LU: c_int = 11;
pub const QN_OPT_LU_PER_COLUMN_PANEL: c_int = 12;
pub const QN_OPT_LU_LOOKAHEAD: c_int = 13;
pub const QN_OPT_LU_ONE_LAUNCH_PANEL: c_int = 14;
pub const QN_OPT_LU_FORCE_WAIT_EXPIRY: c_int = 15;
pub const QN_OPT_CHUNKS_PER_TRIP: c_int = 16;
pub const QN_OPT_LU_SPLIT_ROLE_A: c_int = 17;
pub const QN_OPT_LU_SPLIT_MIN_ROWS: c_int = 18;
pub const QN_OPT_BTB_PROJECT_IN_EVAL: c_int = 19;
pub const QN_OPT_EVAL_ZIGZAG: c_int = 20;
pub const QN_OPT_TOUCH_H_ROWS: c_int = 21;
pub const QN_OPT_TOUCH_Q_ROWS: c_int = 22;
pub const QN_OPT_PNEWTON_REUSE_FACTOR: c_int = 23;
pub const QN_OPT_PNORM_NONTEMPORAL: c_int = 24;
pub const QN_OPT_PNORM_ROWS_PER_WAVE: c_int = 25;
pub const QN_OPT_LBFGS_UNIT_SCALING: c_int = 26;
pub const QN_OPT_MACHINE_FAST_STEPS: c_int = 27;

pub const QN_UNIQUE_ID_BYTES: usize = 128;
pub const QN_TRACE_LS_MODIFIED: i32 = 1 << 30;
pub const QN_PATH_FUSED: u32 = 1;
pub const QN_PATH_SYM: u32 = 2;
pub const QN_PATH_SYM_GENERIC: u32 = 4;
pub const QN_PATH_PIPELINED: u32 = 8;
pub const QN_PATH_SYM2: u32 = 16;
pub const QN_PATH_TILES1: u32 = 32;
pub const QN_PATH_VECTOR: u32 = 64;
pub const QN_PATH_PNEWTON: u32 = 128;
pub const QN_PATH_RANK1: u32 = 256;
pub const QN_PATH_PNORM: u32 = 512;
pub const QN_PATH_LBFGS: u32 = 1024;

#[repr(C)] pub struct qn_context { _p: [u8; 0] }
#[repr(C)] pub struct qn_solver { _p: [u8; 0] }
#[repr(C)] pub struct qn_objective { _p: [u8; 0] }

#[repr(C)]
#[derive(Clone, Copy, Debug)]
pub struct qn_linesearch {
    pub kind: i32,
    pub _pad: i32,
    pub c1: f64,
    pub c2: f64,
    pub t_min: f64,
    pub t_max: f64,
    pub delta_min: f64,
    pub delta: f64,
    pub delta_max: f64,
    pub bt_c1: f64,
    pub bt_beta: f64,
    pub lower_bound_host: *const f64,
    pub upper_bound_host: *const f64,
}

pub type qn_host_oracle_fn = Option<unsafe extern "C" fn(user: *mut c_void, x_host: *const f64, n: usize, f: *mut f64, g_host: *mut f64) -> c_int>;
pub type qn_device_oracle_fn = Option<unsafe extern "C" fn(user: *mut c_void, stream: *mut c_void, x_dev: *const f64, n: usize, f_dev: *mut f64, g_dev: *mut f64) -> c_int>;
pub type qn_host_hessian_fn = Option<unsafe extern "C" fn(user: *mut c_void, x_host: *const f64, n: usize, h_colmajor_host: *mut f64) -> c_int>;
pub type qn_host_allgather_fn = Option<unsafe extern "C" fn(user: *mut c_void, sendbuf: *const f64, recvbuf: *mut f64, count: usize) -> c_int>;
pub type qn_callback_fn = Option<unsafe extern "C" fn(user: *mut c_void, solver: *mut qn_solver)>;

#[repr(C)]
#[derive(Clone, Copy)]
pub struct qn_oracle {
    pub kind: i32,
    pub memoize: i32,
    pub host_fn: qn_host_oracle_fn,
    pub host_user: *mut c_void,
    pub device_fn: qn_device_oracle_fn,
    pub device_user: *mut c_void,
    pub objective: *mut qn_objective,
    pub host_hessian_fn: qn_host_hessian_fn,
}

#[repr(C)]
#[derive(Clone, Copy, Debug, Default)]
pub struct qn_trace_rec {
    pub f: f64,
    pub gnorm: f64,
    pub t: f64,
    pub s_norm: f64,
    pub y_norm: f64,
    pub n_evals: i32,
    pub ls_iters: i32,
    pub ls_cases: i32,
    pub updated: i32,
}

#[repr(C)]
#[derive(Clone, Copy, Debug, Default)]
pub struct qn_stats {
    pub iterations: u64,
    pub oracle_calls: u64,
    pub oracle_evals: u64,
    pub h_passes: u64,
    pub h_bytes: u64,
    pub obj_bytes: u64,
    pub launches: u64,
    pub host_syncs: u64,
    pub t_hpass_ms: f64,
    pub t_eval_ms: f64,
    pub t_ctl_ms: f64,
    pub t_comm_ms: f64,
    pub n_hpass_timed: u64,
    pub n_eval_timed: u64,
    pub n_ctl_timed: u64,
    pub n_comm_timed: u64,
    pub matrix_bytes_per_pass: u64,
    pub total_minimize_calls: u64,
    pub total_iterations: u64,
    pub total_oracle_calls: u64,
    pub total_oracle_evals: u64,
    pub total_h_passes: u64,
    pub total_h_bytes: u64,
    pub total_obj_bytes: u64,
    pub path: u32,
    pub _pad: u32,
    pub t_hreduce_ms: f64,
    pub t_ereduce_ms: f64,
    pub n_hreduce_timed: u64,
    pub n_ereduce_timed: u64,
    pub total_xchg_vector: u64,
    pub total_xchg_scalar: u64,
    pub t_newton_ms: f64,
    pub n_newton_timed: u64,
    pub newton_lu_sync_timeouts: u64,
    pub fast_machine_steps: u64,
}

extern "C" {
    pub fn qn_status_string(status: c_int) -> *const c_char;
    pub fn qn_last_error_message() -> *const c_char;
    pub fn qn_abi_version() -> c_int;

    pub fn qn_device_count(out: *mut c_int) -> c_int;
    pub fn qn_context_create(device: c_int, out: *mut *mut qn_context) -> c_int;
    pub fn qn_comm_unique_id(out_128_bytes: *mut c_void) -> c_int;
    pub fn qn_context_create_sharded(device: c_int, rank: c_int, world: c_int, unique_id: *const c_void, out: *mut *mut qn_context) -> c_int;
    pub fn qn_context_create_sharded_host_exchange(device: c_int, rank: c_int, world: c_int, fn_: qn_host_allgather_fn, user: *mut c_void, out: *mut *mut qn_context) -> c_int;
    pub fn qn_context_set_allreduce(ctx: *mut qn_context, on: c_int) -> c_int;
    pub fn qn_context_set_host_exchange_async(ctx: *mut qn_context, on: c_int) -> c_int;
    pub fn qn_context_set_trial_vector_exchange(ctx: *mut qn_context, on: c_int) -> c_int;
    pub fn qn_context_destroy(ctx: *mut qn_context);
    pub fn qn_partition(n: usize, world: c_int, rows_per_rank: *mut usize, n_pad: *mut usize) -> c_int;
    pub fn qn_comm_selftest(ctx: *mut qn_context) -> c_int;
    pub fn qn_context_comm_check(ctx: *mut qn_context) -> c_int;
    pub fn qn_context_exchange_probe(ctx: *mut qn_context, count: usize, reps: c_int, out_us: *mut f64) -> c_int;
    pub fn qn_context_event_bracket_overhead(ctx: *mut qn_context, reps: c_int, out_ms: *mut f64) -> c_int;
    pub fn qn_context_synchronize(ctx: *mut qn_context) -> c_int;
    pub fn qn_context_rank(ctx: *const qn_context) -> c_int;
    pub fn qn_context_world(ctx: *const qn_context) -> c_int;
    pub fn qn_context_stream(ctx: *mut qn_context) -> *mut c_void;

    pub fn qn_morethuente_default(ls: *mut qn_linesearch);
    pub fn qn_morethuente_with_deltas(ls: *mut qn_linesearch, dmin: f64, d: f64, dmax: f64) -> c_int;
    pub fn qn_morethuente_with_t_min(ls: *mut qn_linesearch, t_min: f64) -> c_int;
    pub fn qn_morethuente_with_t_max(ls: *mut qn_linesearch, t_max: f64) -> c_int;
    pub fn qn_morethuente_with_c1(ls: *mut qn_linesearch, c1: f64) -> c_int;
    pub fn qn_morethuente_with_c2(ls: *mut qn_linesearch, c2: f64) -> c_int;
    pub fn qn_backtracking_new(ls: *mut qn_linesearch, c1: f64, beta: f64);
    pub fn qn_morethuente_b_new(ls: *mut qn_linesearch);
    pub fn qn_backtracking_b_new(ls: *mut qn_linesearch, c1: f64, beta: f64, lower_bound_host: *const f64, upper_bound_host: *const f64);
    pub fn qn_linesearch_with_lower_bound(ls: *mut qn_linesearch, lower_bound_host: *const f64);
    pub fn qn_linesearch_with_upper_bound(ls: *mut qn_linesearch, upper_bound_host: *const f64);
    pub fn qn_nosearch_new(ls: *mut qn_linesearch);
    pub fn qn_gll_quadratic_new(ls: *mut qn_linesearch, c1: f64, m: usize);
    pub fn qn_gll_quadratic_with_sigmas(ls: *mut qn_linesearch, sigma1: f64, sigma2: f64);
    pub fn qn_strong_wolfe_new(ls: *mut qn_linesearch, c1: f64, c2: f64);
    pub fn qn_strong_wolfe_with_xtol(ls: *mut qn_linesearch, xtol: f64) -> c_int;

    pub fn qn_quadratic_create(ctx: *mut qn_context, n: usize, q_rowmajor_host: *const f64, b_host: *const f64, out: *mut *mut qn_objective) -> c_int;
    pub fn qn_quadratic_create_synthetic(ctx: *mut qn_context, n: usize, seed: u64, diag_host: *const f64, b_host: *const f64, out: *mut *mut qn_objective) -> c_int;
    pub fn qn_logsumexp_create(ctx: *mut qn_context, m: usize, n: usize, a_rowmajor_host: *const f64, c_host: *const f64, mu: f64, out: *mut *mut qn_objective) -> c_int;
    pub fn qn_objective_destroy(obj: *mut qn_objective);
    pub fn qn_objective_eval(obj: *mut qn_objective, x_host: *const f64, f: *mut f64, g_host: *mut f64) -> c_int;
    pub fn qn_objective_get_rows(obj: *mut qn_objective, row0: usize, nrows: usize, out_host: *mut f64) -> c_int;
    pub fn qn_objective_hessian(obj: *mut qn_objective, x_host: *const f64, h_colmajor_host: *mut f64) -> c_int;

    pub fn qn_solver_create(ctx: *mut qn_context, method: c_int, tol: f64, x0_host: *const f64, n: usize, out: *mut *mut qn_solver) -> c_int;
    pub fn qn_solver_destroy(s: *mut qn_solver);
    pub fn qn_solver_set_bounds(s: *mut qn_solver, lower_bound_host: *const f64, upper_bound_host: *const f64) -> c_int;
    pub fn qn_solver_set_inverse_p(s: *mut qn_solver, p_colmajor_host: *const f64) -> c_int;
    pub fn qn_solver_get_inverse_p(s: *mut qn_solver, out_colmajor_host: *mut f64) -> c_int;
    pub fn qn_solver_set_spg_lambdas(s: *mut qn_solver, lambda_min: f64, lambda_max: f64) -> c_int;
    pub fn qn_solver_spg_lambda(s: *mut qn_solver, out: *mut f64, is_some: *mut c_int) -> c_int;
    pub fn qn_solver_newton_factorisations(s: *mut qn_solver, out: *mut usize) -> c_int;
    pub fn qn_solver_set_lbfgs_memory(s: *mut qn_solver, m: usize) -> c_int;
    pub fn qn_solver_lbfgs_state(s: *mut qn_solver, m: *mut usize, stored: *mut usize, gamma: *mut f64, resets: *mut usize) -> c_int;
    pub fn qn_solver_reset(s: *mut qn_solver, x0_host: *const f64) -> c_int;
    pub fn qn_minimize(s: *mut qn_solver, ls: *mut qn_linesearch, oracle: *const qn_oracle, max_iter_solver: usize, max_iter_line_search: usize, callback: qn_callback_fn, callback_user: *mut c_void) -> c_int;
    pub fn qn_compute_step_len(ctx: *mut qn_context, ls: *mut qn_linesearch, x_k_host: *const f64, f_k: f64, g_k_host: *const f64, direction_host: *const f64, n: usize, oracle: *const qn_oracle, max_iter: usize, step_out: *mut f64) -> c_int;
    pub fn qn_solver_n(s: *const qn_solver) -> usize;
    pub fn qn_solver_k(s: *const qn_solver) -> usize;
    pub fn qn_solver_set_k(s: *mut qn_solver, k: usize) -> c_int;
    pub fn qn_solver_tol(s: *const qn_solver) -> f64;
    pub fn qn_solver_get_x(s: *mut qn_solver, out_host: *mut f64) -> c_int;
    pub fn qn_solver_set_x(s: *mut qn_solver, x_host: *const f64) -> c_int;
    pub fn qn_solver_s_norm(s: *mut qn_solver, out: *mut f64, is_some: *mut c_int) -> c_int;
    pub fn qn_solver_y_norm(s: *mut qn_solver, out: *mut f64, is_some: *mut c_int) -> c_int;
    pub fn qn_solver_next_iterate_too_close(s: *mut qn_solver, out: *mut c_int) -> c_int;
    pub fn qn_solver_gradient_next_iterate_too_close(s: *mut qn_solver, out: *mut c_int) -> c_int;
    pub fn qn_solver_decrement_squared(s: *mut qn_solver, out: *mut f64, is_some: *mut c_int) -> c_int;
    pub fn qn_solver_get_inv_hessian(s: *mut qn_solver, out_colmajor_host: *mut f64, all_ranks: c_int) -> c_int;
    pub fn qn_solver_set_inv_hessian(s: *mut qn_solver, h_colmajor_host: *const f64) -> c_int;
    pub fn qn_solver_compute_direction(s: *mut qn_solver, g_host: *const f64, d_host: *mut f64) -> c_int;
    pub fn qn_solver_secant_update(s: *mut qn_solver, s_host: *const f64, y_host: *const f64) -> c_int;

    pub fn qn_solver_set_trace(s: *mut qn_solver, cap: usize, with_x: c_int) -> c_int;
    pub fn qn_solver_get_trace(s: *mut qn_solver, out_host: *mut qn_trace_rec, cap: usize, len: *mut usize, x_trace_host: *mut f64) -> c_int;
    pub fn qn_solver_get_stats(s: *mut qn_solver, out: *mut qn_stats) -> c_int;
// ... 16 lines not shown
```

Baseline: 13970.

## Skip H store on alternate passes by deferring two rank-2 updates into one

Adds a store-skip mode for the single-device fused symmetric BFGS path. On alternate H-passes the updated inverse-Hessian tile is not written back. Instead the previous update vectors and coefficients are saved, and the following pass applies both rank-2 updates before storing. This aims to cut the H-matrix write traffic roughly in half, at the cost of extra arithmetic, extra shared memory and saved vectors, and flush logic on export or on path changes.

```diff
diff --git a/include/qn_hip.h b/include/qn_hip.h
--- a/include/qn_hip.h
+++ b/include/qn_hip.h
@@ -190,6 +190,8 @@
     uint64_t n_newton_timed;
     uint64_t newton_lu_sync_timeouts;
     uint64_t fast_machine_steps;
+    uint64_t n_hpass_nostore;
+    uint64_t h_bytes_moved;
 } qn_stats;
 #define QN_PATH_FUSED 1u
 #define QN_PATH_SYM 2u
@@ -233,7 +235,8 @@
     QN_OPT_PNORM_NONTEMPORAL = 24,
     QN_OPT_PNORM_ROWS_PER_WAVE = 25,
     QN_OPT_LBFGS_UNIT_SCALING = 26,
-    QN_OPT_MACHINE_FAST_STEPS = 27
+    QN_OPT_MACHINE_FAST_STEPS = 27,
+    QN_OPT_HPASS_STORE_SKIP = 28
 } qn_option;
 int qn_solver_set_option(qn_solver* s, int option, int value);
 
diff --git a/optimization-solvers_amd/_abi.py b/optimization-solvers_amd/_abi.py
--- a/optimization-solvers_amd/_abi.py
+++ b/optimization-solvers_amd/_abi.py
@@ -59,7 +59,7 @@
                 ("t_hreduce_ms", C.c_double), ("t_ereduce_ms", C.c_double), ("n_hreduce_timed", C.c_uint64), ("n_ereduce_timed", C.c_uint64),
                 ("total_xchg_vector", C.c_uint64), ("total_xchg_scalar", C.c_uint64),
                 ("t_newton_ms", C.c_double), ("n_newton_timed", C.c_uint64), ("newton_lu_sync_timeouts", C.c_uint64),
-                ("fast_machine_steps", C.c_uint64)]
+                ("fast_machine_steps", C.c_uint64), ("n_hpass_nostore", C.c_uint64), ("h_bytes_moved", C.c_uint64)]
 
 
 PATH_FUSED, PATH_SYM, PATH_SYM_GENERIC, PATH_PIPELINED, PATH_SYM2, PATH_TILES1, PATH_VECTOR, PATH_PNEWTON = 1, 2, 4, 8, 16, 32, 64, 128
diff --git a/optimization-solvers_amd/csrc/qn_ctl.h b/optimization-solvers_amd/csrc/qn_ctl.h
--- a/optimization-solvers_amd/csrc/qn_ctl.h
+++ b/optimization-solvers_amd/csrc/qn_ctl.h
@@ -102,6 +102,9 @@
     int32_t pending;
     int32_t spec_tiles;
     double c_ss, c_su, c_uu;
+    double o_ss, o_su, o_uu;
+    int32_t hskip;
+    int32_t hskip_pad;
 
     double f_e, gd_e;
     int32_t last_valid, d_finite;
@@ -119,5 +122,6 @@
     int32_t dir_ready;
 
     uint64_t n_oracle_calls, n_oracle_evals, n_hpasses, n_hpass_rw, n_iterations;
+    uint64_t n_hpass_nostore;
     uint64_t n_fast_steps;
 };
diff --git a/optimization-solvers_amd/csrc/qn_ctl_step.hip.h b/optimization-solvers_amd/csrc/qn_ctl_step.hip.h
--- a/optimization-solvers_amd/csrc/qn_ctl_step.hip.h
+++ b/optimization-solvers_amd/csrc/qn_ctl_step.hip.h
@@ -37,7 +37,7 @@
     c.k = 0;
     if (!c.warm) { c.have_cur_eval = 0; c.have_dir = 0; c.last_valid = 0; c.gg_valid = 0; }
     else c.last_valid = 0;
-    c.n_oracle_calls = 0; c.n_oracle_evals = 0; c.n_hpasses = 0; c.n_hpass_rw = 0; c.n_iterations = 0;
+    c.n_oracle_calls = 0; c.n_oracle_evals = 0; c.n_hpasses = 0; c.n_hpass_rw = 0; c.n_hpass_nostore = 0; c.n_iterations = 0;
     c.status = -1;
     c.state = QN_ST_LOOP_TOP;
 }
@@ -123,10 +123,16 @@
     const double yu = c.hp_yu;
     double c_ss, c_su, c_uu;
     qn_update_coeffs(c.method, c.ys, yu, c_ss, c_su, c_uu, c.hp_den);
-    c.c_ss = c_ss; c.c_su = c_su; c.c_uu = c_uu;
     c.n_hpasses++;
     if (c.pending) c.n_hpass_rw++;
-    c.pending = 1;
+    if (c.hskip && c.pending == 1) {
+        c.o_ss = c.c_ss; c.o_su = c.c_su; c.o_uu = c.c_uu;
+        c.pending = 2;
+        c.n_hpass_nostore++;
+    } else {
+        c.pending = 1;
+    }
+    c.c_ss = c_ss; c.c_su = c_su; c.c_uu = c_uu;
     c.sc ^= 1;
     c.dir_mode = 1; c.dir_ug = c.hp_ug; c.dir_sg = c.hp_sg;
     c.gd0_valid = 0; c.d_finite = 0;
diff --git a/optimization-solvers_amd/csrc/qn_host_launch.hip.h b/optimization-solvers_amd/csrc/qn_host_launch.hip.h
--- a/optimization-solvers_amd/csrc/qn_host_launch.hip.h
+++ b/optimization-solvers_amd/csrc/qn_host_launch.hip.h
@@ -362,7 +362,7 @@
     QnCtl* pc = s->hrep;
     memcpy(pc, s->hctl, sizeof(QnCtl));
     pc->phase = QN_PH_REQ_HPASS; pc->serviced = 0; pc->hp_nrhs = 1; pc->pending = 0; pc->after_state = QN_ST_AFTER_DIR; pc->sym2 = 1; pc->fused = 1;
-    pc->spec_tiles = 0; pc->sc = 0; pc->xc = 0;
+    pc->spec_tiles = 0; pc->sc = 0; pc->xc = 0; pc->hskip = 0;
     PinnedBuf<QnCtl> pe;
     (void)pe.alloc(1, hipHostMallocMapped | hipHostMallocCoherent);
     if (pe) {
diff --git a/optimization-solvers_amd/csrc/qn_host_minimize.hip.h b/optimization-solvers_amd/csrc/qn_host_minimize.hip.h
--- a/optimization-solvers_amd/csrc/qn_host_minimize.hip.h
+++ b/optimization-solvers_amd/csrc/qn_host_minimize.hip.h
@@ -88,6 +88,8 @@
     }
     r.sym2 = r.sym && (s2_shape || s2sh_shape);
     h->sym2 = r.sym2 ? 1 : 0;
+    h->hskip = 0;
+    if (!r.sym2) QNCHK(flush_older(s));
     r.bnd = r.sym2 && (s->bounded || ls_bounded || s->method == QN_SR1);
     if ((s->bounded || ls_bounded) && r.fused && !r.bnd) return fail(QN_ABNORMAL_TERMINATION, "bounded run on a fused path that is not the second-generation one");
     if (s->method == QN_SR1 && r.fused && !r.sym2) return fail(QN_ABNORMAL_TERMINATION, "SR1 on a fused path that is not the second-generation one");
@@ -195,6 +197,13 @@
     s2_cache_policy(c->world > 1 ? (size_t)s->T.rpr * s->T.n_pad * 8 / 2 : (size_t)s->T.n_pad * s->T.n_pad * 8 / 2, &a.nt, &a.ntq);
     if (getenv("QN_S2_NT")) a.nt = atoi(getenv("QN_S2_NT"));
     if (getenv("QN_S2_NTQ")) a.ntq = atoi(getenv("QN_S2_NTQ"));
+    {
+        QnCtl* h = s->hctl;
+        const bool skip = s->hpass_skip && c->world == 1 && !r.gobj && !r.bnd && !r.tiles1 && !a.fold && !a.tred && s->method != QN_SR1;
+        if (!skip) QNCHK(flush_older(s));
+        h->hskip = skip ? 1 : 0;
+        a.so = fused_so(s); a.uo = fused_uo(s);
+    }
     return QN_OK;
 }
 
@@ -363,6 +372,7 @@
     s->stats.oracle_evals = h->n_oracle_evals;
     s->stats.h_passes = h->n_hpasses;
     s->stats.fast_machine_steps = h->n_fast_steps;
+    s->stats.n_hpass_nostore = h->n_hpass_nostore;
     uint64_t shard = (uint64_t)s->T.rpr * (uint64_t)s->T.n_pad * 8ull;
     const uint64_t full_shard = shard;
     if (r.sym || r.sym_generic) shard = (uint64_t)s->sym_nb * (uint64_t)(s->sym_nb + 1) / 2ull * (uint64_t)QN_TB * QN_TB * 8ull;
@@ -376,6 +386,7 @@
     }
     s->stats.h_bytes = (h->n_hpasses + h->n_hpass_rw) * shard;
     if (r.sym2) s->stats.h_bytes = 2 * h->n_hpasses * shard;
+    s->stats.h_bytes_moved = s->stats.h_bytes - h->n_hpass_nostore * shard;
     s->stats.obj_bytes = (r.oracle_tpl == QN_ORACLE_QUAD) ? h->n_oracle_evals * (r.sym ? shard : full_shard) : 0;
     if (r.obj && r.obj->kind == OBJ_LOGSUMEXP)
         s->stats.obj_bytes = h->n_oracle_evals * (uint64_t)r.obj->TA.rpr * (uint64_t)r.obj->T.n_pad * 8ull * ((r.obj->lse_kch && !r.obj->lse_two_pass) ? 1ull : 2ull);
diff --git a/optimization-solvers_amd/csrc/qn_host_solver.hip.h b/optimization-solvers_amd/csrc/qn_host_solver.hip.h
--- a/optimization-solvers_amd/csrc/qn_host_solver.hip.h
+++ b/optimization-solvers_amd/csrc/qn_host_solver.hip.h
@@ -37,6 +37,7 @@
     bool no_pair = false;
     int ring = (getenv("QN_S2_RING") && atoi(getenv("QN_S2_RING")) == 0) ? 0 : 1;
     int zig = (getenv("QN_S2_ZIGZAG") && atoi(getenv("QN_S2_ZIGZAG")) == 0) ? 0 : 1;
+    int hpass_skip = 1;
     int fast_steps = 1;
     int touch = getenv("QN_S2_TOUCH") ? atoi(getenv("QN_S2_TOUCH")) : 8;
     int touchq = getenv("QN_S2_TOUCHQ") ? atoi(getenv("QN_S2_TOUCHQ")) : 6;
@@ -171,7 +172,7 @@
 static int solver_alloc_fused(qn_solver* s, bool sym) {
     const size_t np = s->T.n_pad;
     hipStream_t st = s->ctx->stream;
-    QNCHK(s->fused_block.ensure(10 * np, st));
+    QNCHK(s->fused_block.ensure(12 * np, st));
     const int nblk = sym ? (int)(np / QN_TB) : s->T.rpr / s->R;
     if (sym) {
         QNCHK(s->sym_part.ensure((size_t)nblk * nblk * 2 * QN_TB, st));
@@ -465,6 +466,7 @@
     case QN_OPT_BTB_PROJECT_IN_EVAL: s->no_projfold = !on; return QN_OK;
     case QN_OPT_EVAL_ZIGZAG: s->zig = on ? 1 : 0; return QN_OK;
     case QN_OPT_MACHINE_FAST_STEPS: s->fast_steps = on ? 1 : 0; return QN_OK;
+    case QN_OPT_HPASS_STORE_SKIP: s->hpass_skip = on ? 1 : 0; return QN_OK;
     case QN_OPT_PNEWTON_REUSE_FACTOR: s->pn_reuse = on ? 1 : 0; s->pn_factor_serial = 0; return QN_OK;
     case QN_OPT_LBFGS_UNIT_SCALING:
         if (s->method != QN_LBFGS) return fail(QN_ERROR_INPUT_PARAMS, "unit scaling belongs to an L-BFGS solver");
@@ -513,8 +515,27 @@
 extern "C" size_t qn_solver_k(const qn_solver* s) { return (size_t)s->hctl->k; }
 extern "C" double qn_solver_tol(const qn_solver* s) { return s->tol; }
 
+static double* fused_so(qn_solver* s) { return (double*)s->fused_block + 10 * (size_t)s->T.n_pad; }
+static double* fused_uo(qn_solver* s) { return (double*)s->fused_block + 11 * (size_t)s->T.n_pad; }
+static int ensure_full_h(qn_solver* s);
+static int launch_hpass_R(qn_solver* s, const QnHPassArgs& a);
+static QnHPassArgs hpass_args(qn_solver* s, int expect_phase);
+static int poke_ctl(qn_solver* s);
+static int flush_older(qn_solver* s) {
+    if (s->hctl->pending != 2) return QN_OK;
+    QNCHK(ensure_full_h(s));
+    QnHPassArgs a = hpass_args(s, -1);
+    a.sp = fused_so(s); a.up = fused_uo(s);
+    a.force_nrhs = 0; a.force_pending = 1;
+    a.c_ss = s->hctl->o_ss; a.c_su = s->hctl->o_su; a.c_uu = s->hctl->o_uu;
+    QNCHK(launch_hpass_R(s, a));
+    s->hctl->pending = 1;
+    return poke_ctl(s);
+}
+
 static int fused_export(qn_solver* s) {
     s->warm_obj = 0;
+    QNCHK(flush_older(s));
     if (!s->fused_live) return QN_OK;
     qn_context* c = s->ctx;
     const QnCtl* h = s->hctl;
diff --git a/optimization-solvers_amd/csrc/qn_sym2.hip.h b/optimization-solvers_amd/csrc/qn_sym2.hip.h
--- a/optimization-solvers_amd/csrc/qn_sym2.hip.h
+++ b/optimization-solvers_amd/csrc/qn_sym2.hip.h
@@ -73,6 +73,7 @@
     int slot;
     int swz;
 #endif
+    double *so, *uo;
 };
 #ifdef QN_S2_STAMPS
 #define QN_S2_WG(a) ((int)blockIdx.x ^ (a).swz)
@@ -1040,6 +1041,9 @@
     QnS2HVec v0;
     double s1_r, y_r;
     v2d s1_c, y_c;
+    constexpr bool PLAIN = !FOLD && !SHARD && !TRED && !SR1;
+    __shared__ v2d wo_c[2][PLAIN ? QN_S2_TPB : 1];
+    __shared__ double wo_r[2][PLAIN ? QN_S2_TPB : 1];
     auto vec_spec = [&]() {
         const int ir = I * QN_TB + wave * QN_S2_RPW + (lane & 15), jc = J * QN_TB + qn_s2_col(I == J, lane, wave);
         QnS2HReq spec;
@@ -1124,8 +1128,19 @@
     const bool fold = FOLD && mine == 2;
     QnS2HReq q;
     bool nrhs2;
+    bool two = false, nost = false;
+    double o_ss = 0.0, o_su = 0.0, o_uu = 0.0;
     {
         const QnCtl& c = L.c;
+        if (PLAIN) {
+            two = __builtin_amdgcn_readfirstlane(c.pending == 2) != 0;
+            nost = __builtin_amdgcn_readfirstlane(c.hskip != 0 && c.pending == 1 && c.hp_nrhs == 2) != 0;
+            o_ss = c.o_ss; o_su = c.o_su; o_uu = c.o_uu;
+            if (two) {
+                const int ir = I * QN_TB + wave * QN_S2_RPW + (lane & 15), jc = J * QN_TB + qn_s2_col(I == J, lane, wave);
+                wo_r[0][tid] = a.so[ir]; wo_r[1][tid] = a.uo[ir]; wo_c[0][tid] = ld2(a.so + jc); wo_c[1][tid] = ld2(a.uo + jc);
+            }
+        }
         q.pending = c.pending != 0;
         q.c_ss = c.c_ss; q.c_su = c.c_su; q.c_uu = c.c_uu;
         q.sp = a.F.S0 + (size_t)c.sc * np;
@@ -1190,10 +1205,28 @@
         const size_t rstride = has_next ? np : 0;
         double c0x = 0.0, c0y = 0.0, c1x = 0.0, c1y = 0.0;
         double racc[QN_S2_RPW];
+        auto rows = [&](auto two_c, auto st_c) __attribute__((always_inline)) {
+        constexpr bool TWO = decltype(two_c)::value, ST = decltype(st_c)::value;
+        double sro = 0.0, uro = 0.0;
+        v2d sjo = {0.0, 0.0}, ujo = {0.0, 0.0};
+        if constexpr (TWO) { sro = wo_r[0][PLAIN ? tid : 0]; uro = wo_r[1][PLAIN ? tid : 0]; sjo = wo_c[0][PLAIN ? tid : 0]; ujo = wo_c[1][PLAIN ? tid : 0]; }
 #pragma unroll
         for (int r = 0; r < QN_S2_RPW; ++r) {
             v2d hn = h[r];
             h[r] = qn_sym_ld<NT>(hnext + (size_t)r * rstride);
+            if constexpr (TWO) {
+                const double si = qn_lane_bcast(sro, r), ui = qn_lane_bcast(uro, r);
+                if (BFGS || SR1) {
+                    hn.x = hn.x + o_su * (si * ujo.x + ui * sjo.x);
+                    hn.y = hn.y + o_su * (si * ujo.y + ui * sjo.y);
+                }
+                hn.x = hn.x + o_ss * (si * sjo.x);
+                hn.y = hn.y + o_ss * (si * sjo.y);
+                if (!BFGS || SR1) {
+                    hn.x = hn.x + o_uu * (ui * ujo.x);
+                    hn.y = hn.y + o_uu * (ui * ujo.y);
+                }
+            }
             const double si = qn_lane_bcast(sr, r), ui = qn_lane_bcast(ur, r);
             if (BFGS || SR1) {
                 hn.x = hn.x + c_su * (si * uj.x + ui * sj.x);
@@ -1205,7 +1238,7 @@
                 hn.x = hn.x + c_uu * (ui * uj.x);
                 hn.y = hn.y + c_uu * (ui * uj.y);
             }
-            qn_sym_st<NT>(hbase + (size_t)r * np, hn);
+            if constexpr (ST) qn_sym_st<NT>(hbase + (size_t)r * np, hn);
             const double y0 = qn_lane_bcast(y0r, r), y1 = qn_lane_bcast(y1r, r);
             double t0 = hn.x * a0.x;
             t0 = __builtin_fma(hn.y, a0.y, t0);
@@ -1221,10 +1254,19 @@
             c1x = __builtin_fma(hn.x, y1, c1x);
             c1y = __builtin_fma(hn.y, y1, c1y);
         }
+        };
+        if constexpr (PLAIN) {
+            if (two) rows(std::true_type{}, std::true_type{});
+            else if (nost) rows(std::false_type{}, std::false_type{});
+            else rows(std::false_type{}, std::true_type{});
+        } else rows(std::false_type{}, std::true_type{});
         if (!qn_s2_col_on(diag, lane, wave)) { c0x = 0.0; c0y = 0.0; c1x = 0.0; c1y = 0.0; }
+        double nso_r = 0.0, nuo_r = 0.0;
+        v2d nso_c = {0.0, 0.0}, nuo_c = {0.0, 0.0};
         if (has_next) {
             const int irn = In * QN_TB + wave * QN_S2_RPW + (lane & 15), ccn = qn_s2_col(In == Jn, lane, wave);
             qn_s2_hvec_load<!FOLD>(q, irn, Jn * QN_TB + ccn, v0);
+            if (PLAIN && two) { nso_r = a.so[irn]; nuo_r = a.uo[irn]; nso_c = ld2(a.so + Jn * QN_TB + ccn); nuo_c = ld2(a.uo + Jn * QN_TB + ccn); }
             if (FOLD) {
                 const int rr = wave * QN_S2_RPW + (lane & 15), bI = 2 * (it + 1), bJ = bI + 1;
                 v0.y0_r = fv[bI][0][rr]; v0.y1_r = fv[bI][1][rr];
@@ -1235,6 +1277,7 @@
             unsigned r = sl.D * QN_TB + sl.row, c = sl.D * QN_TB + 2 * lane;
             asm volatile("" : "+v"(r), "+v"(c));
             qn_s2_hvec_load<true>(q, r, c, v0);
+            if (PLAIN && two) { nso_r = a.so[r]; nuo_r = a.uo[r]; nso_c = ld2(a.so + c); nuo_c = ld2(a.uo + c); }
         }
         if (it == 0) { qn_keepalive(racc[0]); QN_S2_STAMP(3); QN_S2_STAMP_T(12, 448); }
         if (it == 1) { qn_keepalive(racc[0]); QN_S2_STAMP(6); QN_S2_STAMP_T(13, 448); }
@@ -1258,12 +1301,27 @@
             else qn_s2_slot_st<TRED>(a.part + (unsigned)(((J * a.nb + I) * 2 + crhs) * QN_TB + c), acc);
         }
         if (it == 0) QN_S2_STAMP(5);
+        if (PLAIN && two) { wo_r[0][PLAIN ? tid : 0] = nso_r; wo_r[1][PLAIN ? tid : 0] = nuo_r; wo_c[0][PLAIN ? tid : 0] = nso_c; wo_c[1][PLAIN ? tid : 0] = nuo_c; }
         if (!has_next) break;
         I = In; J = Jn; hbase = hnext;
         __syncthreads();
     }
     if (slv) {
         v2d hn = h[0];
+        if (PLAIN && two) {
+            const double si = wo_r[0][PLAIN ? tid : 0], ui = wo_r[1][PLAIN ? tid : 0];
+            const v2d sjo = wo_c[0][PLAIN ? tid : 0], ujo = wo_c[1][PLAIN ? tid : 0];
+            if (BFGS || SR1) {
+                hn.x = hn.x + o_su * (si * ujo.x + ui * sjo.x);
+                hn.y = hn.y + o_su * (si * ujo.y + ui * sjo.y);
+            }
+            hn.x = hn.x + o_ss * (si * sjo.x);
+            hn.y = hn.y + o_ss * (si * sjo.y);
+            if (!BFGS || SR1) {
+                hn.x = hn.x + o_uu * (ui * ujo.x);
+                hn.y = hn.y + o_uu * (ui * ujo.y);
+            }
+        }
         const double si = pend ? v0.s_r : 0.0, ui = pend ? v0.u_r : 0.0;
         v2d sj = {0.0, 0.0}, uj = {0.0, 0.0};
         if (pend) { sj = v0.s_c; uj = v0.u_c; }
@@ -1277,7 +1335,7 @@
             hn.x = hn.x + c_uu * (ui * uj.x);
             hn.y = hn.y + c_uu * (ui * uj.y);
         }
-        qn_sym_st<NT>(sliver_ptr(), hn);
+        if (!nost) qn_sym_st<NT>(sliver_ptr(), hn);
         double t0 = hn.x * v0.a0.x;
         t0 = __builtin_fma(hn.y, v0.a0.y, t0);
         double t1 = hn.x * v0.a1.x;
@@ -1385,6 +1443,7 @@
     QnS2Slots S0;
     QN_S2_STAMP(0);
     double gp = 0.0, yv = 0.0, s0e = 0.0, s1e = 0.0;
+    constexpr bool PLAIN = !SHARD && !SR1;
     auto entries = [&]() {
         if (half != 1 && tid < QN_TB) {
             gp = a.F.GT[R * QN_TB + tid]; yv = a.F.Y[R * QN_TB + tid];
@@ -1402,6 +1461,11 @@
     double tot0 = 0.0, tot1 = 0.0;
     if (!SHARD) {
         if (half == 1 && nrhs != 2) return;
+        if (PLAIN && L.c.hskip && L.c.pending == 1 && nrhs == 2 && tid < QN_TB) {
+            const int gi = R * QN_TB + tid;
+            if (half == 0) a.uo[gi] = a.F.UN[gi];
+            else a.so[gi] = a.F.S0[(size_t)(L.c.sc ? a.np : 0) + gi];
+        }
         const double t = qn_s2_slot_sum(a.part, a.nb, R, half, S0, qbuf);
         if (half == 0) tot0 = t; else tot1 = t;
     } else if (tid < QN_TB) {
diff --git a/optimization-solvers_amd/solver.py b/optimization-solvers_amd/solver.py
--- a/optimization-solvers_amd/solver.py
+++ b/optimization-solvers_amd/solver.py
@@ -47,6 +47,7 @@
     "pnorm_rows_per_wave": 25,
     "lbfgs_unit_scaling": 26,
     "machine_fast_steps": 27,
+    "hpass_store_skip": 28,
 }
 OPT_GENERIC_KERNELS = 1
 OPT_DEFERRED_UPDATE_STEP = 2
@@ -75,6 +76,7 @@
 OPT_PNORM_ROWS_PER_WAVE = 25
 OPT_LBFGS_UNIT_SCALING = 26
 OPT_MACHINE_FAST_STEPS = 27
+OPT_HPASS_STORE_SKIP = 28
 
 
 class SolverError(Exception):
diff --git a/rust/src/ffi.rs b/rust/src/ffi.rs
--- a/rust/src/ffi.rs
+++ b/rust/src/ffi.rs
@@ -63,6 +63,7 @@
 pub const QN_OPT_PNORM_ROWS_PER_WAVE: c_int = 25;
 pub const QN_OPT_LBFGS_UNIT_SCALING: c_int = 26;
 pub const QN_OPT_MACHINE_FAST_STEPS: c_int = 27;
+pub const QN_OPT_HPASS_STORE_SKIP: c_int = 28;
 
 pub const QN_UNIQUE_ID_BYTES: usize = 128;
 pub const QN_TRACE_LS_MODIFIED: i32 = 1 << 30;
@@ -172,6 +173,8 @@
     pub n_newton_timed: u64,
     pub newton_lu_sync_timeouts: u64,
     pub fast_machine_steps: u64,
+    pub n_hpass_nostore: u64,
+    pub h_bytes_moved: u64,
 }
 
 extern "C" {
```

Result: faster. 14190, median of 6 (+1.6%).
